# EricSteinberger/PokerRL

Measured on NVIDIA H100. Metric: CFR+ iterations/s, higher is better.
Workload: dtype f32

## Files before the change

### include/pokerrl_b200.h

```cpp
#ifndef POKERRL_B200_H
#define POKERRL_B200_H

#include <stdint.h>

#ifdef __cplusplus
extern "C" {
#endif

typedef void* prl_stream_t;

#define PRL_ABI_VERSION 10

enum {
    PRL_KIND_P0 = 0,
    PRL_KIND_P1 = 1,
    PRL_KIND_CHANCE = 2,
    PRL_KIND_FOLD = 3,
    PRL_KIND_SHOWDOWN = 4,
    PRL_KIND_SHOWDOWN_ALLIN = 5
};

enum { PRL_ALGO_VANILLA = 0, PRL_ALGO_CFR_PLUS = 1, PRL_ALGO_LINEAR = 2, PRL_ALGO_DCFR = 3, PRL_ALGO_PCFR_PLUS = 4 };

enum {
    PRL_STRAT_F32 = 0,
    PRL_STRAT_UNIFORM64 = 1,
    PRL_STRAT_AVG_F64 = 2,
    PRL_STRAT_AVG_SUM = 3,
    PRL_STRAT_AVG_F32 = 4
};

typedef struct {
    int32_t n_nodes, n_levels, n_slots;
    int32_t n_range;
    int32_t ld;
    int32_t n_hole;
    int32_t n_deck;
    int32_t n_suits;
    int32_t pair_bonus;
    int32_t max_actions;
    const int64_t* level_start;
    const int32_t* parent;
    const int32_t* first_child;
    const int32_t* n_children;
    const int32_t* slot;
    const int8_t* kind;
    const int8_t* acted_last;
    const float* pot;
    const int32_t* board;
    const int32_t* order;
    const int64_t* level_nonterm;
    const void* meta;
    const int64_t* level_ndec;
    const int8_t* hand_cards;
    int32_t n_boards;
    int32_t max_chance_children;
    const uint64_t* board_mask;
    const float* board_prob;
    const float* board_mult;
    const int16_t* board_gs;
    const int16_t* board_ge;
    const int16_t* board_pos;
    const int16_t* board_row_order;
    const uint8_t* board_row_pos;
    const uint8_t* board_complete;
    int32_t n_sym;
    const int16_t* sym_perm;
    float eq_const;
    const void* board_hand_rec;
    const void* node_rec2;
    const void* work_rec2;
    const int64_t* level_nfold;
    const int64_t* level_nallin;
    const int32_t* allin_nodes;
    const float* allin_pot;
    const void* const* allin_tiles;
    float* allin_partial;
} prl_tree_t;

typedef struct {
    float* reach;
    float* ev;
    float* ev_br;
    float* regret;
    float* strat;
    void* avg;
    void* workspace;
    uint64_t workspace_bytes;
    const float* dcfr;
} prl_buffers_t;

int prl_abi_version(void);
const char* prl_last_error(void);
unsigned long long prl_launch_count(void);

int prl_pack_node_meta(const prl_tree_t* tree, void* out_meta, prl_stream_t stream);

int prl_reach_pass(const prl_tree_t* tree, const prl_buffers_t* buf, int player_mask, const int* strat_mode,
                   prl_stream_t stream);

int prl_value_pass(const prl_tree_t* tree, const prl_buffers_t* buf, int player_mask, int with_br,
                   const int* strat_mode, prl_stream_t stream);

int prl_root_exploitability(const prl_tree_t* tree, const prl_buffers_t* buf, float* out_expl, prl_stream_t stream);

int prl_cfr_half_iteration(const prl_tree_t* tree, const prl_buffers_t* buf, int algo, int p, int iter, int delay,
                           int avg_f64, const int* strat_mode, prl_stream_t stream);

int prl_cfr_iterations(const prl_tree_t* tree, const prl_buffers_t* buf, int algo, int iter0, int n_iters, int delay,
                       int avg_f64, const int* strat_mode, prl_stream_t stream);

int prl_evaluate(const prl_tree_t* tree, const prl_buffers_t* buf, const int* strat_mode, int do_reach, float* out_expl,
                 prl_stream_t stream);

void prl_debug_set_timeline(void* device_u64_buffer);

int prl_cfr_sweep(const prl_tree_t* tree, const prl_buffers_t* buf, int algo, int p, int iter, int delay, int avg_f64,
                  const int* strat_mode, int which, prl_stream_t stream);

int prl_value_levels(const prl_tree_t* tree, const prl_buffers_t* buf, int player_mask, int with_br, int algo, int upd_p,
                     int iter, int delay, const int* strat_mode, int level_hi, int level_lo, int chance_phase,
                     prl_stream_t stream);
int prl_reach_update(const prl_tree_t* tree, const prl_buffers_t* buf, int algo, int p, int iter, int delay,
                     prl_stream_t stream);

int prl_reach_levels(const prl_tree_t* tree, const prl_buffers_t* buf, int player_mask, int algo, int upd_p, int iter,
                     int delay, const int* strat_mode, int level_lo, int level_hi, prl_stream_t stream);

int prl_gather_agent_policy(const float* probs, int n_actions, const int32_t* dec_of_slot, const int32_t* action_of_slot,
                            int n_slots, int n_range, int ld, float* out, prl_stream_t stream);

int prl_board_order_tables(const int32_t* ranks, int n_boards, int n_range, int n_deck, int16_t* gs, int16_t* ge,
                           int16_t* pos, int16_t* row_order, uint8_t* row_pos, prl_stream_t stream);

typedef struct {
    int32_t n_boards;
    int32_t n_range;
    int32_t ld;
    int32_t n_deck;
    int32_t n_local;
    int32_t frac_bits;
    int32_t grid;
    float eq_const;
    int8_t kind[16], parent[16], first_child[16], n_children[16], acted_last[16];
    float pot[16];
    int64_t row0[16];
    int32_t row_m[16];
    const void* tables;
    const float* board_prob;
    const float* board_mult;
    float* regret;
    float* avg;
    int64_t* w_private;
    int64_t* w_total;
    const float* dcfr;
    float* pred;
    float* rnr_reach;
    float rnr_p;
} prl_board_game_t;

int prl_board_layout(const prl_board_game_t* shape, int32_t* out);
int prl_board_grid(void);
int prl_board_shape_ok(const prl_board_game_t* g);
int prl_board_rows(const prl_board_game_t* shape, int32_t* row_of, int32_t* rows_per_board);

int prl_board_build_tables(const int32_t* ranks, const uint64_t* board_mask, const int8_t* hand_cards, int n_boards,
                           void* blob, prl_stream_t stream);

int prl_board_sweep(const prl_board_game_t* g, int p, int eval, int src_own, int src_opp, const float* trunk_reach_opp,
                    int iter, int delay, int algo, float defer_w, int p1_only, prl_stream_t stream);

int prl_board_update_cfrp(const prl_board_game_t* g, int p, const float* trunk_reach_opp, int iter, int delay, int due, int now,
                          prl_stream_t stream);
int prl_board_avg_flush(const prl_board_game_t* g, int p, int due, int delay, prl_stream_t stream);

int prl_board_collect(const prl_board_game_t* g, int n_arr, const int16_t* sym_perm, int n_sym, float* out, int ld,
                      prl_stream_t stream);

typedef struct {
    int32_t n_nodes, chance_node, n_buf_nodes, ld, n_range;
    int32_t mode[2];
    float eq_const;
    int8_t kind[8], first_child[8], n_children[8], acted_last[8];
    int32_t first_slot[8];
    float pot[8];
    const int8_t* hand_cards;
    float* reach;
    float* ev;
    float* ev_br;
    float* regret;
    float* strat;
    float* avg;
    const float* reach_model;
    float rnr_p;
} prl_trunk_t;

int prl_board_trunk(const prl_board_game_t* g, const prl_trunk_t* t, int eval, int p, int n_sym, const int16_t* sym_perm, int iter,
                    int delay, float* out_expl, const int64_t* const* peers, int n_peers, int64_t peer_offset, int64_t* w_scratch,
                    int algo, prl_stream_t stream);

int prl_board_permute(const prl_board_game_t* g, int rows_per_board, const int64_t* row_src, const int64_t* row_dst,
                      float* sorted_tab, float* natural_tab, int ld, int to_natural, prl_stream_t stream);

int prl_board_policy_query(const prl_board_game_t* shape, const float* rows, const int64_t* keys, const int16_t* pos_hand,
                           int n_cls, int iso, const int8_t* boards, int n_boards, const int32_t* out_index, uint64_t actions,
                           int n_actions, float* out, int32_t* miss, prl_stream_t stream);


int64_t prl_allin_tiles_bytes(int n_range);
int64_t prl_allin_partial_bytes(int n_range);
int prl_allin_equity_accumulate(const int32_t* ranks, const double* weight, int n_boards, int n_range, double* ec,
                                prl_stream_t stream);
int prl_allin_equity_finish(const double* ec, int n_range, const int8_t* hand_cards, const int16_t* sym_perm, int n_sym,
                            void* tiles, prl_stream_t stream);
int prl_allin_values(const void* tiles, int n_range, const float* const* x_rows, float* const* y_rows, float* const* y2_rows,
                     const float* scale, int n_cols, float* partial, prl_stream_t stream);

int prl_hand_rank_boards(const int8_t* boards, int n_boards, int32_t* out, prl_stream_t stream);

int prl_hand_rank_7(const int8_t* cards, int n, int32_t* out, prl_stream_t stream);

long long prl_lbr_workspace_doubles(int n_queries, int n_dealt);
int prl_lbr_checkdown_equity(const int8_t* lbr_hands, const int8_t* boards, int n_dealt, const float* ranges, int n_queries,
                             int first_board_ranks, double* workspace, float* out, prl_stream_t stream);

int32_t get_hand_rank_52_holdem(int8_t** hand_2d , int8_t** board_2d );
void get_hand_rank_all_hands_on_given_boards_52_holdem(int32_t** out , int8_t** boards_1d ,
                                                       int32_t n, int8_t** idx2holecards, int8_t** card1d_to_2d);
void get_hole_card_2_idx_lut(int16_t** lut );
void get_idx_2_hole_card_lut(int8_t** lut );
void get_idx_2_flop_lut(int8_t** lut );
void get_idx_2_turn_lut(int8_t** lut );
void get_idx_2_river_lut(int8_t** lut );
int8_t get_1d_card(const int8_t* card_2d);
void get_2d_card(int8_t card_1d, int8_t* out_card_2d);

#define PRL_ENV_MAX_ACTIONS 34

typedef struct {
    int32_t n_envs;
    int32_t kind;
    int32_t n_actions;
    int32_t n_rounds;
    int32_t n_round_slots;
    int32_t n_hole, n_ranks, n_suits, n_deck;
    int32_t n_flop, n_turn, n_river;
    int32_t small_blind, big_blind, ante, small_bet, big_bet, round_big_bet_starts;
    int32_t max_raises[4];
    int32_t first_action_no_call, limit_raise_is_pot, btn_first_postflop, suits_matter;
    int32_t pair_bonus;
    int32_t start_stack[2];
    int32_t obs_size;
    double fracs[32];
    double reward_scalar;
    double norm;
} prl_env_cfg_t;

int prl_env_state_fields(void);

int prl_env_reset(const prl_env_cfg_t* cfg, int32_t* state, int8_t* deck, float* obs, uint8_t* legal, uint64_t seed,
                  uint64_t episode0, int shuffle, prl_stream_t stream);

int prl_env_step(const prl_env_cfg_t* cfg, int32_t* state, int8_t* deck, const int32_t* actions, float* obs,
                 double* rewards, uint8_t* done, uint8_t* legal, uint64_t seed, uint64_t step_id, int auto_reset,
                 prl_stream_t stream);

#ifdef __cplusplus
}
#endif
#endif
```

### pokerrl_b200/_native.py

```python
import ctypes as C
import os

_HERE = os.path.dirname(os.path.abspath(__file__))
LIB_PATH = os.environ.get("PRL_LIB_PATH") or os.path.join(_HERE, "lib", "libpokerrl_b200.so")

KIND_P0, KIND_P1, KIND_CHANCE, KIND_FOLD, KIND_SHOWDOWN, KIND_SHOWDOWN_ALLIN = range(6)
ALGO_VANILLA, ALGO_CFR_PLUS, ALGO_LINEAR, ALGO_DCFR, ALGO_PCFR_PLUS = 0, 1, 2, 3, 4
ABI_VERSION = 10
STRAT_F32, STRAT_UNIFORM64, STRAT_AVG_F64, STRAT_AVG_SUM, STRAT_AVG_F32 = range(5)


class PrlTree(C.Structure):
    _fields_ = [
        ("n_nodes", C.c_int32), ("n_levels", C.c_int32), ("n_slots", C.c_int32), ("n_range", C.c_int32),
        ("ld", C.c_int32), ("n_hole", C.c_int32), ("n_deck", C.c_int32), ("n_suits", C.c_int32),
        ("pair_bonus", C.c_int32), ("max_actions", C.c_int32),
        ("level_start", C.c_void_p),
        ("parent", C.c_void_p), ("first_child", C.c_void_p), ("n_children", C.c_void_p), ("slot", C.c_void_p),
        ("kind", C.c_void_p), ("acted_last", C.c_void_p), ("pot", C.c_void_p), ("board", C.c_void_p),
        ("order", C.c_void_p), ("level_nonterm", C.c_void_p), ("meta", C.c_void_p),
        ("level_ndec", C.c_void_p), ("hand_cards", C.c_void_p), ("n_boards", C.c_int32),
        ("max_chance_children", C.c_int32), ("board_mask", C.c_void_p), ("board_prob", C.c_void_p),
        ("board_mult", C.c_void_p), ("board_gs", C.c_void_p), ("board_ge", C.c_void_p), ("board_pos", C.c_void_p),
        ("board_row_order", C.c_void_p), ("board_row_pos", C.c_void_p), ("board_complete", C.c_void_p),
        ("n_sym", C.c_int32), ("sym_perm", C.c_void_p), ("eq_const", C.c_float), ("board_hand_rec", C.c_void_p),
        ("node_rec2", C.c_void_p), ("work_rec2", C.c_void_p), ("level_nfold", C.c_void_p),
        ("level_nallin", C.c_void_p), ("allin_nodes", C.c_void_p), ("allin_pot", C.c_void_p), ("allin_tiles", C.c_void_p),
        ("allin_partial", C.c_void_p),
    ]


class PrlBuffers(C.Structure):
    _fields_ = [("reach", C.c_void_p), ("ev", C.c_void_p), ("ev_br", C.c_void_p), ("regret", C.c_void_p),
                ("strat", C.c_void_p), ("avg", C.c_void_p), ("workspace", C.c_void_p),
                ("workspace_bytes", C.c_uint64), ("dcfr", C.c_void_p)]


class PrlBoardGame(C.Structure):
    _fields_ = [("n_boards", C.c_int32), ("n_range", C.c_int32), ("ld", C.c_int32), ("n_deck", C.c_int32),
                ("n_local", C.c_int32), ("frac_bits", C.c_int32), ("grid", C.c_int32), ("eq_const", C.c_float),
                ("kind", C.c_int8 * 16), ("parent", C.c_int8 * 16), ("first_child", C.c_int8 * 16),
                ("n_children", C.c_int8 * 16), ("acted_last", C.c_int8 * 16), ("pot", C.c_float * 16),
                ("row0", C.c_int64 * 16), ("row_m", C.c_int32 * 16),
                ("tables", C.c_void_p), ("board_prob", C.c_void_p), ("board_mult", C.c_void_p), ("regret", C.c_void_p),
                ("avg", C.c_void_p), ("w_private", C.c_void_p), ("w_total", C.c_void_p), ("dcfr", C.c_void_p), ("pred", C.c_void_p),
                ("rnr_reach", C.c_void_p), ("rnr_p", C.c_float)]


class PrlTrunk(C.Structure):
    _fields_ = [("n_nodes", C.c_int32), ("chance_node", C.c_int32), ("n_buf_nodes", C.c_int32), ("ld", C.c_int32),
                ("n_range", C.c_int32), ("mode", C.c_int32 * 2), ("eq_const", C.c_float),
                ("kind", C.c_int8 * 8), ("first_child", C.c_int8 * 8), ("n_children", C.c_int8 * 8), ("acted_last", C.c_int8 * 8),
                ("first_slot", C.c_int32 * 8), ("pot", C.c_float * 8), ("hand_cards", C.c_void_p), ("reach", C.c_void_p),
                ("ev", C.c_void_p), ("ev_br", C.c_void_p), ("regret", C.c_void_p), ("strat", C.c_void_p), ("avg", C.c_void_p),
                ("reach_model", C.c_void_p), ("rnr_p", C.c_float)]


class PrlEnvCfg(C.Structure):
    _fields_ = [
        ("n_envs", C.c_int32), ("kind", C.c_int32), ("n_actions", C.c_int32), ("n_rounds", C.c_int32),
        ("n_round_slots", C.c_int32), ("n_hole", C.c_int32), ("n_ranks", C.c_int32), ("n_suits", C.c_int32),
        ("n_deck", C.c_int32), ("n_flop", C.c_int32), ("n_turn", C.c_int32), ("n_river", C.c_int32),
        ("small_blind", C.c_int32), ("big_blind", C.c_int32), ("ante", C.c_int32), ("small_bet", C.c_int32),
        ("big_bet", C.c_int32), ("round_big_bet_starts", C.c_int32), ("max_raises", C.c_int32 * 4),
        ("first_action_no_call", C.c_int32), ("limit_raise_is_pot", C.c_int32), ("btn_first_postflop", C.c_int32),
        ("suits_matter", C.c_int32), ("pair_bonus", C.c_int32), ("start_stack", C.c_int32 * 2), ("obs_size", C.c_int32),
        ("fracs", C.c_double * 32), ("reward_scalar", C.c_double), ("norm", C.c_double),
    ]


_lib = None


def lib():
    global _lib
    if _lib is not None:
        return _lib
    if not os.path.exists(LIB_PATH):
        raise RuntimeError(
            "pokerrl_b200: CUDA library %s is missing. Build it with `python -m pokerrl_b200.csrc.build` "
            "(or __graft_entry__.build()). There is no CPU fallback." % LIB_PATH)
    L = C.CDLL(LIB_PATH)
    L.prl_abi_version.restype = C.c_int
    if L.prl_abi_version() != ABI_VERSION:
        raise RuntimeError("pokerrl_b200: %s was built for ABI %d, the Python side expects %d - rebuild it with "
                           "`python -m pokerrl_b200.csrc.build`" % (LIB_PATH, L.prl_abi_version(), ABI_VERSION))
    L.prl_last_error.restype = C.c_char_p
    tp, bp, ip = C.POINTER(PrlTree), C.POINTER(PrlBuffers), C.POINTER(C.c_int)
    L.prl_reach_pass.argtypes = [tp, bp, C.c_int, ip, C.c_void_p]
    L.prl_value_pass.argtypes = [tp, bp, C.c_int, C.c_int, ip, C.c_void_p]
    L.prl_root_exploitability.argtypes = [tp, bp, C.c_void_p, C.c_void_p]
    L.prl_cfr_half_iteration.argtypes = [tp, bp, C.c_int, C.c_int, C.c_int, C.c_int, C.c_int, ip, C.c_void_p]
    L.prl_cfr_sweep.argtypes = [tp, bp, C.c_int, C.c_int, C.c_int, C.c_int, C.c_int, ip, C.c_int, C.c_void_p]
    L.prl_launch_count.restype = C.c_ulonglong
    L.prl_cfr_iterations.argtypes = [tp, bp, C.c_int, C.c_int, C.c_int, C.c_int, C.c_int, ip, C.c_void_p]
    L.prl_evaluate.argtypes = [tp, bp, ip, C.c_int, C.c_void_p, C.c_void_p]
    L.prl_pack_node_meta.argtypes = [tp, C.c_void_p, C.c_void_p]
    for f in ("prl_reach_pass", "prl_value_pass", "prl_root_exploitability", "prl_cfr_half_iteration", "prl_cfr_sweep", "prl_pack_node_meta", "prl_cfr_iterations",
              "prl_evaluate"):
        getattr(L, f).restype = C.c_int
    L.prl_value_levels.argtypes = [tp, bp, C.c_int, C.c_int, C.c_int, C.c_int, C.c_int, C.c_int, ip, C.c_int, C.c_int,
                                   C.c_int, C.c_void_p]
    L.prl_reach_update.argtypes = [tp, bp, C.c_int, C.c_int, C.c_int, C.c_int, C.c_void_p]
    L.prl_value_levels.restype = L.prl_reach_update.restype = C.c_int
    L.prl_reach_levels.argtypes = [tp, bp, C.c_int, C.c_int, C.c_int, C.c_int, C.c_int, ip, C.c_int, C.c_int, C.c_void_p]
    L.prl_reach_levels.restype = C.c_int
    L.prl_board_order_tables.argtypes = [C.c_void_p, C.c_int, C.c_int, C.c_int, C.c_void_p, C.c_void_p, C.c_void_p,
                                         C.c_void_p, C.c_void_p, C.c_void_p]
    L.prl_board_order_tables.restype = C.c_int
    L.prl_hand_rank_boards.argtypes = [C.c_void_p, C.c_int, C.c_void_p, C.c_void_p]
    L.prl_hand_rank_7.argtypes = [C.c_void_p, C.c_int, C.c_void_p, C.c_void_p]
    for f in ("prl_hand_rank_boards", "prl_hand_rank_7"):
        getattr(L, f).restype = C.c_int
    L.prl_gather_agent_policy.argtypes = [C.c_void_p, C.c_int, C.c_void_p, C.c_void_p, C.c_int, C.c_int, C.c_int, C.c_void_p,
                                          C.c_void_p]
    L.prl_gather_agent_policy.restype = C.c_int
    L.prl_lbr_workspace_doubles.argtypes = [C.c_int, C.c_int]
    L.prl_lbr_workspace_doubles.restype = C.c_longlong
    L.prl_lbr_checkdown_equity.argtypes = [C.c_void_p, C.c_void_p, C.c_int, C.c_void_p, C.c_int, C.c_int, C.c_void_p, C.c_void_p,
                                           C.c_void_p]
    L.prl_lbr_checkdown_equity.restype = C.c_int
    L.prl_allin_tiles_bytes.argtypes = L.prl_allin_partial_bytes.argtypes = [C.c_int]
    L.prl_allin_tiles_bytes.restype = L.prl_allin_partial_bytes.restype = C.c_int64
    L.prl_allin_equity_accumulate.argtypes = [C.c_void_p, C.c_void_p, C.c_int, C.c_int, C.c_void_p, C.c_void_p]
    L.prl_allin_equity_finish.argtypes = [C.c_void_p, C.c_int, C.c_void_p, C.c_void_p, C.c_int, C.c_void_p, C.c_void_p]
    L.prl_allin_values.argtypes = [C.c_void_p, C.c_int, C.c_void_p, C.c_void_p, C.c_void_p, C.c_void_p, C.c_int, C.c_void_p,
                                   C.c_void_p]
    for f in ("prl_allin_equity_accumulate", "prl_allin_equity_finish", "prl_allin_values"):
        getattr(L, f).restype = C.c_int
    gp = C.POINTER(PrlBoardGame)
    L.prl_board_layout.argtypes = [gp, C.POINTER(C.c_int32)]
    L.prl_board_grid.argtypes = []
    L.prl_board_rows.argtypes = [gp, C.POINTER(C.c_int32), C.POINTER(C.c_int32)]
    L.prl_board_rows.restype = C.c_int
    L.prl_board_shape_ok.argtypes = [gp]
    L.prl_board_build_tables.argtypes = [C.c_void_p, C.c_void_p, C.c_void_p, C.c_int, C.c_void_p, C.c_void_p]
    L.prl_board_sweep.argtypes = [gp, C.c_int, C.c_int, C.c_int, C.c_int, C.c_void_p, C.c_int, C.c_int, C.c_int, C.c_float, C.c_int,
                                  C.c_void_p]
    L.prl_board_update_cfrp.argtypes = [gp, C.c_int, C.c_void_p, C.c_int, C.c_int, C.c_int, C.c_int, C.c_void_p]
    L.prl_board_avg_flush.argtypes = [gp, C.c_int, C.c_int, C.c_int, C.c_void_p]
    L.prl_board_collect.argtypes = [gp, C.c_int, C.c_void_p, C.c_int, C.c_void_p, C.c_int, C.c_void_p]
    L.prl_board_permute.argtypes = [gp, C.c_int, C.c_void_p, C.c_void_p, C.c_void_p, C.c_void_p, C.c_int, C.c_int,
                                    C.c_void_p]
    L.prl_board_trunk.argtypes = [gp, C.POINTER(PrlTrunk), C.c_int, C.c_int, C.c_int, C.c_void_p, C.c_int, C.c_int, C.c_void_p,
                                  C.c_void_p, C.c_int, C.c_int64, C.c_void_p, C.c_int, C.c_void_p]
    L.prl_board_trunk.restype = C.c_int
    L.prl_board_policy_query.argtypes = [gp, C.c_void_p, C.c_void_p, C.c_void_p, C.c_int, C.c_int, C.c_void_p, C.c_int,
                                         C.c_void_p, C.c_uint64, C.c_int, C.c_void_p, C.c_void_p, C.c_void_p]
    for f in ("prl_board_layout", "prl_board_grid", "prl_board_shape_ok", "prl_board_build_tables", "prl_board_sweep",
              "prl_board_update_cfrp", "prl_board_avg_flush", "prl_board_collect", "prl_board_permute", "prl_board_policy_query"):
        getattr(L, f).restype = C.c_int
    ep = C.POINTER(PrlEnvCfg)
    L.prl_env_state_fields.restype = C.c_int
    L.prl_env_reset.argtypes = [ep, C.c_void_p, C.c_void_p, C.c_void_p, C.c_void_p, C.c_uint64, C.c_uint64, C.c_int,
                                C.c_void_p]
    L.prl_env_step.argtypes = [ep, C.c_void_p, C.c_void_p, C.c_void_p, C.c_void_p, C.c_void_p, C.c_void_p, C.c_void_p,
                               C.c_uint64, C.c_uint64, C.c_int, C.c_void_p]
    L.prl_env_reset.restype = L.prl_env_step.restype = C.c_int
    _lib = L
    return L


def call(name, *args):
    L = lib()
    rc = getattr(L, name)(*args)
    if rc != 0:
        raise RuntimeError("%s failed (%d): %s" % (name, rc, L.prl_last_error().decode()))


def modes(m0, m1):
    return (C.c_int * 2)(m0, m1)
```

### pokerrl_b200/board_engine.py

```python
import ctypes as C
import math
import os

import numpy as np
import torch

from pokerrl_b200 import _native as nat
from pokerrl_b200 import algorithm
from pokerrl_b200 import dcfr as _dcfr
from pokerrl_b200.game.flat_tree import FlatTree
from pokerrl_b200.game.holdem_boards import BoardSpec
from pokerrl_b200.solver import DeviceTree, TreeBuffers, TreeOps, _require_cuda

SRC_REGRET, SRC_AVG, SRC_AVG_SUM = 0, 1, 2


def board_layout(g=None):
    out = (C.c_int32 * 8)()
    nat.call("prl_board_layout", C.byref(g) if g is not None else None, out)
    return dict(n_live=out[0], ldb=out[1], blob=out[2], sh_off=out[3], rows_off=out[4], live_cards=out[5],
                row_pad=out[6], n_local=out[7])


def _stream(dev):
    return C.c_void_p(torch.cuda.current_stream(dev).cuda_stream)


def supports(game_cls, env_args, algo):
    if algo not in algorithm.ALL or game_cls.RULES.N_HOLE_CARDS != 2 or game_cls.RULES.N_CARDS_IN_DECK != 52:
        return False
    if game_cls.RULES.N_FLOP_CARDS != 5 or os.environ.get("PRL_ENGINE", "board") != "board":
        return False
    try:
        ft1 = FlatTree(game_cls, env_args, board_spec=_one_board_spec())
    except Exception:
        return False
    st = ft1.board_subtree()
    if st is None or sum(1 for n in ft1.abs_nodes if n.kind == nat.KIND_CHANCE) != 1:
        return False
    g = nat.PrlBoardGame()
    _fill_shape(g, st)
    return bool(nat.lib().prl_board_shape_ok(C.byref(g)))


def _one_board_spec():
    return BoardSpec(np.array([[0, 1, 2, 3, 4]], np.int8), np.ones(1), np.ones(1), None, "shape probe")


def _fill_shape(g, st):
    g.n_local = st["n_local"]
    for i in range(st["n_local"]):
        g.kind[i], g.parent[i], g.first_child[i] = st["kind"][i], st["parent"][i], st["first_child"][i]
        g.n_children[i], g.acted_last[i], g.pot[i] = st["n_children"][i], st["acted_last"][i], st["pot"][i]


def shape_rows(g):
    row_of, rpb = (C.c_int32 * 16)(), C.c_int32(0)
    nat.call("prl_board_rows", C.byref(g), row_of, C.byref(rpb))
    return list(row_of), int(rpb.value)


def board_mask(boards):
    mask = np.zeros(boards.shape[0], np.uint64)
    for k in range(boards.shape[1]):
        mask |= (np.uint64(1) << boards[:, k].astype(np.uint64))
    return mask


def build_board_blobs(rules, boards, t_blob, dev):
    from pokerrl_b200.hand_eval import hand_rank_all_hands_on_given_boards
    boards = np.ascontiguousarray(boards, np.int8)
    nb = boards.shape[0]
    lut = rules.get_lut_holder()
    t_hc = torch.from_numpy(np.ascontiguousarray(lut.LUT_IDX_2_HOLE_CARDS, np.int8)).to(dev)
    t_mask = torch.from_numpy(board_mask(boards).view(np.int64)).to(dev)
    CH = 16384
    for i in range(0, nb, CH):
        n = min(CH, nb - i)
        ranks = hand_rank_all_hands_on_given_boards(boards[i:i + n], device=dev)
        nat.call("prl_board_build_tables", C.c_void_p(ranks.data_ptr()), C.c_void_p(t_mask[i:i + n].data_ptr()),
                 C.c_void_p(t_hc.data_ptr()), n, C.c_void_p(t_blob[i:i + n].data_ptr()), _stream(dev))


def _decision_locals(st):
    return [i for i in range(st["n_local"]) if st["kind"][i] <= 1 and st["n_children"][i] > 0]


def board_game(st, rules, n_boards, ld, n_sym, grid=0):
    g = nat.PrlBoardGame()
    _fill_shape(g, st)
    g.n_boards, g.n_range, g.ld, g.n_deck = n_boards, rules.RANGE_SIZE, ld, rules.N_CARDS_IN_DECK
    n_hole = rules.N_HOLE_CARDS
    g.eq_const = math.comb(g.n_deck, n_hole) / math.comb(g.n_deck - n_hole, n_hole)
    bound = max(n_sym, 1) * g.eq_const * max(st["pot"]) * 0.5 * 4.0
    g.frac_bits = 62 - int(math.ceil(math.log2(bound)))
    n_local = st["n_local"]
    dec = _decision_locals(st)
    rows_per_board = sum(st["n_children"][i] for i in dec)
    row_of, rpb = shape_rows(g)
    assert rpb == rows_per_board
    local_rows = {}
    for i in range(n_local):
        g.row0[i], g.row_m[i] = -1, 0
    for d in dec:
        for a in range(st["n_children"][d]):
            c = st["first_child"][d] + a
            g.row0[c], g.row_m[c] = row_of[c], rpb
            local_rows[c] = (int(row_of[c]), rpb)
    g.grid = int(grid) if grid else int(nat.lib().prl_board_grid())
    return g, rows_per_board, local_rows


def row_map(local_rows, ft=None):
    st = None if ft is None else ft.board_subtree()
    src, dst = [], []
    for k, (i, (r0, m)) in enumerate(sorted(local_rows.items())):
        src += [r0, m]
        dst += [k, len(local_rows)] if ft is None else [int(ft.slot[st["node_base"][i] + st["node_k"][i]]), st["node_m"][i]]
    return src, dst


def _normalised(x, dim, matching):
    if matching:
        x = x.clamp(min=0)
    tot = x.sum(dim=dim, keepdim=True)
    ok = (tot > 0) if matching else (tot != 0)
    return torch.where(ok, x / torch.where(ok, tot, torch.ones_like(tot)), torch.full_like(x, 1.0 / x.shape[dim]))


def _sum_to_one(x, dim):
    d = x.double()
    tot = d.sum(dim=dim, keepdim=True)
    ok = tot > 0
    return torch.where(ok, d / torch.where(ok, tot, torch.ones_like(tot)), torch.full_like(d, 1.0 / d.shape[dim])).to(x.dtype)


def _decision_row_groups(st, local_rows):
    return [[local_rows[c][0] for c in range(st["first_child"][d], st["first_child"][d] + st["n_children"][d])]
            for d in _decision_locals(st)]


def _trunk_decisions(ft, chance_node):
    return [(int(ft.first_slot[n]), int(ft.n_children[n])) for n in range(chance_node + 1)
            if ft.kind[n] <= 1 and ft.first_child[n] >= 0]


class _BoardEngine:

    def _setup(self, game_cls, env_args, spec, n_boards, grid=0):
        dev = self.device
        self.rules = game_cls.RULES
        self.ev_normalizer = game_cls.EV_NORMALIZER
        self.L = board_layout()
        self.ft1 = FlatTree(game_cls, env_args, board_spec=_one_board_spec())
        st = self.ft1.board_subtree()
        if st is None:
            raise ValueError("the game does not have ONE chance layer with a <= 16-node post-deal subtree")
        self.st = st
        self.chance_level = st["chance_level"]
        self.chance_node = st["chance_node"]
        self.R = self.rules.RANGE_SIZE
        self.trunk = DeviceTree(self.ft1, dev)
        self.trunk.desc.n_sym = 0
        self.trunk.desc.sym_perm = None
        self.bufs = TreeBuffers(self.trunk)
        self.ld = self.trunk.ld
        sp = spec.sym_perm
        self.n_sym = 0 if sp is None else int(sp.shape[0])
        self.t_sym = None if sp is None else torch.from_numpy(np.ascontiguousarray(sp, np.int16)).to(dev)
        g, self.rows_per_board, self.local_rows = board_game(st, self.rules, n_boards, self.ld, self.n_sym, grid)
        self.w_private = torch.zeros((g.grid, 2, self.R), dtype=torch.int64, device=dev)
        self._expl = torch.zeros(2, dtype=torch.float32, device=dev)
        g.w_private = self.w_private.data_ptr()
        self.g = g
        nb = self.n_boards_total = int(spec.boards.shape[0])
        self.n_nodes = int(self.ft1.level_start[self.chance_level + 1]) + nb * st["n_local"]
        self.n_nonterm = (int((self.ft1.kind[:self.chance_node + 1] <= nat.KIND_CHANCE).sum())
                          + nb * len(_decision_locals(st)))

    def _setup_boards(self, capacity):
        dev, n = self.device, max(capacity, 1)
        self.t_blob = torch.empty((n, self.L["blob"]), dtype=torch.uint8, device=dev)
        self.t_prob = torch.zeros(n, dtype=torch.float32, device=dev)
        self.t_mult = torch.zeros(n, dtype=torch.float32, device=dev)
        g = self.g
        g.tables, g.board_prob, g.board_mult = self.t_blob.data_ptr(), self.t_prob.data_ptr(), self.t_mult.data_ptr()

    def _load_boards(self, boards, prob, mult):
        n = boards.shape[0]
        build_board_blobs(self.rules, boards, self.t_blob, self.device)
        self.t_prob[:n].copy_(torch.from_numpy(np.ascontiguousarray(prob, np.float32)))
        self.t_mult[:n].copy_(torch.from_numpy(np.ascontiguousarray(mult, np.float32)))
        self.g.n_boards = n

    def _trunk_desc(self, bufs, modes):
        ft, t = self.ft1, nat.PrlTrunk()
        n = self.chance_node + 1
        assert n <= 8 and int(ft.level_start[self.chance_level + 1]) == n, "the trunk must be the first nodes of the flat tree"
        t.n_nodes, t.chance_node, t.n_buf_nodes, t.ld, t.n_range = n, self.chance_node, self.trunk.n_nodes, self.ld, self.R
        t.mode[0], t.mode[1] = modes
        t.eq_const = self.g.eq_const
        for i in range(n):
            t.kind[i], t.first_child[i], t.n_children[i] = int(ft.kind[i]), int(ft.first_child[i]), int(ft.n_children[i])
            t.acted_last[i], t.pot[i] = int(ft.acted_last[i]), float(ft.pot[i])
            t.first_slot[i] = int(ft.first_slot[i]) if ft.first_slot[i] >= 0 else 0
        t.hand_cards = self.trunk.t_hand_cards.data_ptr()
        t.reach, t.ev, t.ev_br = bufs.reach.data_ptr(), bufs.ev.data_ptr(), bufs.ev_br.data_ptr()
        t.regret, t.strat, t.avg = bufs.regret.data_ptr(), bufs.strat.data_ptr(), bufs.avg.data_ptr()
        return t

    def _trunk_reach_row(self, bufs, seat):
        return C.c_void_p(bufs.reach.data_ptr() + 4 * (seat * self.trunk.n_nodes + self.chance_node) * self.ld)

    def _reach_trunk(self, bufs, mask, algo, upd_p, modes, t, delay):
        nat.call("prl_reach_levels", C.byref(self.trunk.desc), C.byref(bufs.desc), mask, algo, upd_p, t, delay,
                 nat.modes(*modes), 0, self.chance_level, _stream(self.device))

    @property
    def n_trunk_slots(self):
        return self.ft1.n_slots - self.rows_per_board

    def _board_sweep(self, bufs, p, evaluate, src_own, src_opp, t, delay, algo, defer_w=0.0, p1_only=0):
        nat.call("prl_board_sweep", C.byref(self.g), p, int(evaluate), src_own, src_opp, self._trunk_reach_row(bufs, 1 - p),
                 t, delay, algo, defer_w, p1_only, _stream(self.device))

    def _board_trunk(self, bufs, modes, evaluate, p, t, delay, algo, peers=None, n_peers=0, peer_off=0, w_scratch=None):
        nat.call("prl_board_trunk", C.byref(self.g), C.byref(self._trunk_desc(bufs, modes)), int(evaluate), p, self.n_sym,
                 C.c_void_p(self.t_sym.data_ptr()) if self.n_sym else None, t, delay, C.c_void_p(self._expl.data_ptr()), peers,
                 n_peers, peer_off, w_scratch, algo, _stream(self.device))

    def _board_permute(self, tab, nat_tab, to_natural, ft=None, lo=0, hi=None):
        g = self.g
        if hi is not None:
            g = nat.PrlBoardGame.from_buffer_copy(self.g)
            g.n_boards, g.tables = hi - lo, self.t_blob[lo].data_ptr()
        src, dst = (torch.tensor(x, dtype=torch.int64, device=self.device) for x in row_map(self.local_rows, ft))
        nat.call("prl_board_permute", C.byref(g), len(self.local_rows), C.c_void_p(src.data_ptr()), C.c_void_p(dst.data_ptr()),
                 C.c_void_p(tab[lo * self.rows_per_board].data_ptr()), C.c_void_p(nat_tab.data_ptr()), self.ld, to_natural,
                 _stream(self.device))


class BoardCFRSolver(_BoardEngine):
    def __init__(self, game_cls, env_args, board_spec=None, algo="CFRPlus", delay=0, device=None, rank=0, world=1,
                 group=None, grid=0, reduce_fn=None, dcfr=_dcfr.DEFAULT, pcfr_gamma=algorithm.PCFR_GAMMA):
        self.device = _require_cuda(device)
        self.alg = algorithm.Algorithm(algo, delay, dcfr, self.device, pcfr_gamma)
        self.algo_name, self.algo, self.delay, self.dcfr = self.alg.name, self.alg.code, self.alg.delay, self.alg.dcfr
        self._factors = self.alg.factors
        self.rank, self.world, self.group = int(rank), int(world), group
        self._reduce_fn = reduce_fn
        self.game_cls, self.env_args = game_cls, env_args
        spec = board_spec if board_spec is not None else BoardSpec.full_game(game_cls.RULES)
        self.spec_full = spec
        with torch.cuda.device(self.device):
            self._build(spec, grid)
        self.n_allreduce = 0
        self.reset()

    def _build(self, spec, grid):
        dev = self.device
        sel = np.arange(self.rank, spec.boards.shape[0], self.world)
        self.board_ids = sel
        self.boards = np.ascontiguousarray(spec.boards[sel], np.int8)
        nb = self.n_boards = int(sel.size)
        self._setup(self.game_cls, self.env_args, spec, nb, grid)
        self.ops = TreeOps(self.trunk, self.bufs)
        self._eval_bufs = None
        self._setup_boards(nb)
        self._load_boards(self.boards, spec.board_prob[sel], spec.board_mult[sel])
        torch.cuda.synchronize(dev)
        g = self.g
        self.n_rows = nb * self.rows_per_board
        self.regret = torch.zeros((max(self.n_rows, 1), self.L["ldb"]), dtype=torch.float32, device=dev)
        self.avg = torch.zeros_like(self.regret)
        g.regret, g.avg = self.regret.data_ptr(), self.avg.data_ptr()
        self.pred = torch.zeros_like(self.regret) if self.algo == nat.ALGO_PCFR_PLUS else None
        g.pred = self.pred.data_ptr() if self.pred is not None else None
        self._symm = None
        self.collective = "none" if self.world == 1 else "nccl all_reduce(int64)"
        if (self.world > 1 and self._reduce_fn is None and os.environ.get("PRL_COLLECTIVE", "p2p") == "p2p"
                and os.environ.get("PRL_TRUNK", "fused") != "levels"):
            try:
                import torch.distributed as dist
                import torch.distributed._symmetric_memory as symm_mem
                self.w_gens = symm_mem.empty((2, 4, self.R), dtype=torch.int64, device=dev)
                self.w_gens.zero_()
                self._symm = symm_mem.rendezvous(self.w_gens, group=self.group if self.group is not None else dist.group.WORLD)
                self._peer_ptrs = torch.tensor([int(x) for x in self._symm.buffer_ptrs], dtype=torch.int64, device=dev)
                self.collective = "one-shot NVLink sum inside trunk_kernel (symmetric memory, %d peers)" % self.world
            except Exception as e:
                self._symm = None
                self.collective = "nccl all_reduce(int64) (symmetric memory unavailable: %s)" % type(e).__name__
        if self._symm is None:
            self.w_gens = torch.zeros((2, 4, self.R), dtype=torch.int64, device=dev)
        self._gen = 0
        self.w_total = self.w_gens[0]
        self.w_scratch = torch.zeros((4, self.R), dtype=torch.int64, device=dev)
        g.w_total = self.w_total.data_ptr()
        self.fused_trunk = os.environ.get("PRL_TRUNK", "fused") != "levels"
        self._w_off = 4 * self.ld

    def _clear_pending(self):
        self._pending = [0.0, 0.0]
        self._avg_due = [-1, -1]

    def _trunk(self, bufs, modes, evaluate, p):
        peers, n_peers, off = None, 0, 0
        if self._symm is not None:
            peers, n_peers, off = C.c_void_p(self._peer_ptrs.data_ptr()), self.world, self._gen * 4 * self.R
        self._board_trunk(bufs, modes, evaluate, p, self.iter_counter, self.delay, self.algo, peers, n_peers, off,
                          C.c_void_p(self.w_scratch.data_ptr()))

    def _board_update_cfrp(self, p, due, now):
        nat.call("prl_board_update_cfrp", C.byref(self.g), p, self._trunk_reach_row(self.bufs, 1 - p), self.iter_counter,
                 self.delay, due, now, _stream(self.device))

    def _next_generation(self):
        self._gen ^= 1
        self.w_total = self.w_gens[self._gen]
        self.g.w_total = self.w_total.data_ptr()

    def _reduce(self, view):
        if self._symm is not None:
            self._symm.barrier(channel=0)
            self.n_allreduce += 1
            return
        if self._reduce_fn is not None:
            self._reduce_fn(view)
        elif self.world > 1:
            import torch.distributed as dist
            dist.all_reduce(view, op=dist.ReduceOp.SUM, group=self.group)
        self.n_allreduce += 1

    def _levels(self, bufs, mask, with_br, algo, upd_p, modes, hi, lo, phase):
        nat.call("prl_value_levels", C.byref(self.trunk.desc), C.byref(bufs.desc), mask, int(with_br), algo, upd_p,
                 self.iter_counter, self.delay, nat.modes(*modes), hi, lo, phase, _stream(self.device))

    def _sweep_begin(self, bufs, p, evaluate, src_own, src_opp):
        if not evaluate and self.algo == nat.ALGO_CFR_PLUS:
            t, due = self.iter_counter, self._avg_due[p]
            now = 1 if due >= 0 or t < self.delay else 0
            self._avg_due[p] = -1 if now else t
            self._board_update_cfrp(p, due, now)
            return
        defer_w = 0.0
        if not evaluate and self.algo != nat.ALGO_CFR_PLUS:
            defer_w, self._pending[1 - p] = self._pending[1 - p], 0.0
        self._board_sweep(bufs, p, evaluate, src_own, src_opp, self.iter_counter, self.delay, self.algo, defer_w)

    def flush_average(self):
        with torch.cuda.device(self.device):
            for q in (0, 1):
                if self._avg_due[q] >= 0:
                    nat.call("prl_board_avg_flush", C.byref(self.g), q, self._avg_due[q], self.delay, _stream(self.device))
                    self._avg_due[q] = -1
                if self._pending[q] != 0.0:
                    self._board_sweep(self.bufs, 1 - q, False, 0, 0, self.iter_counter, self.delay, self.algo,
                                      defer_w=self._pending[q], p1_only=1)
                    self._pending[q] = 0.0

    def _sweep_end(self, bufs, p, evaluate):
        n_arr = 2 if evaluate else 1
        view = self.w_total[2 * p:2 * p + 2] if evaluate else self.w_total[:1]
        self._reduce(view)
        out = bufs.workspace.data_ptr() + 4 * (self._w_off + 2 * p * self.ld)
        g2 = self.g
        if evaluate and p == 1:
            g2 = nat.PrlBoardGame.from_buffer_copy(self.g)
            g2.w_total = self.w_total.data_ptr() + 8 * 2 * self.R
        nat.call("prl_board_collect", C.byref(g2), n_arr, C.c_void_p(self.t_sym.data_ptr()) if self.n_sym else None,
                 self.n_sym, C.c_void_p(out), self.ld, _stream(self.device))

    def _sweep(self, bufs, p, evaluate, src_own, src_opp):
        self._sweep_begin(bufs, p, evaluate, src_own, src_opp)
        self._sweep_end(bufs, p, evaluate)

    def _update_begin(self, p):
        cl = self.chance_level
        self.g.dcfr = self.alg.factor_table(self.iter_counter + 1)
        if not self.fused_trunk:
            self._levels(self.bufs, 1 << p, False, self.algo, p, self.modes, cl, cl, 1)
        self._sweep_begin(self.bufs, p, False, SRC_REGRET, SRC_REGRET)

    def _update_end(self, p):
        cl = self.chance_level
        if self.algo != nat.ALGO_CFR_PLUS:
            if not self.fused_trunk:
                raise RuntimeError("Vanilla / Linear CFR, DCFR and PCFR+ on the board engine need the fused trunk (unset "
                                   "PRL_TRUNK=levels)")
            self._pending[p] = self.alg.sum_weight(self.iter_counter)
        if self.fused_trunk:
            self._reduce(self.w_total[:1])
            self._trunk(self.bufs, self.modes, False, p)
            self.modes[p] = nat.STRAT_F32
            self._next_generation()
            return
        self._sweep_end(self.bufs, p, False)
        self._levels(self.bufs, 1 << p, False, self.algo, p, self.modes, cl, cl, 2)
        if cl > 0:
            self._levels(self.bufs, 1 << p, False, self.algo, p, self.modes, cl - 1, 0, 0)
        self.modes[p] = nat.STRAT_F32
        self._reach_trunk(self.bufs, 1 << p, self.algo, p, self.modes, self.iter_counter, self.delay)

    def reset(self):
        with torch.cuda.device(self.device):
            self.iter_counter = 0
            for t in (self.regret, self.avg, self.bufs.regret, self.bufs.strat, self.bufs.avg):
                t.zero_()
            if self.pred is not None:
                self.pred.zero_()
            self._clear_pending()
            self.modes = [nat.STRAT_UNIFORM64, nat.STRAT_UNIFORM64]
            self._reach_trunk(self.bufs, 3, -1, -1, self.modes, self.iter_counter, self.delay)

    def iteration(self, n=1):
        with torch.cuda.device(self.device):
            for _ in range(n):
                for p in (0, 1):
                    self._update_begin(p)
                    self._update_end(p)
                self.iter_counter += 1

    def _evaluate(self, bufs, modes, src):
        cl = self.chance_level
        if self.fused_trunk:
            for p in (0, 1):
                self._sweep_begin(bufs, p, True, src, src)
            self._reduce(self.w_total)
            self._trunk(bufs, modes, True, -1)
            self._next_generation()
            e = self._expl.cpu().numpy()
        else:
            self._levels(bufs, 3, True, -1, -1, modes, cl, cl, 1)
            for p in (0, 1):
                self._sweep(bufs, p, True, src, src)
            self._levels(bufs, 3, True, -1, -1, modes, cl, cl, 2)
            if cl > 0:
                self._levels(bufs, 3, True, -1, -1, modes, cl - 1, 0, 0)
            e = (TreeOps(self.trunk, bufs) if bufs is not self.bufs else self.ops).root_exploitability()
        return algorithm.seat_averaged(e, self.ev_normalizer)

    def exploitability_current(self):
        with torch.cuda.device(self.device):
            return self._evaluate(self.bufs, self.modes, SRC_REGRET)

    def exploitability_average(self):
        if self.iter_counter == 0:
            raise RuntimeError("no average strategy before the first iteration")
        m, src = {algorithm.SUMS: (nat.STRAT_AVG_SUM, SRC_AVG_SUM), algorithm.CURRENT: (nat.STRAT_F32, SRC_REGRET),
                  algorithm.AVERAGE: (nat.STRAT_AVG_F32, SRC_AVG)}[self.alg.average(self.iter_counter)]
        with torch.cuda.device(self.device):
            if self._eval_bufs is None:
                self._eval_bufs = TreeBuffers(self.trunk, share=self.bufs)
            self.flush_average()
            self._reach_trunk(self._eval_bufs, 3, -1, -1, [m, m], self.iter_counter, self.delay)
            return self._evaluate(self._eval_bufs, [m, m], src)

    def natural_tables(self, ft):
        assert ft.board_spec.boards.shape[0] == self.n_boards
        self.flush_average()
        nts, out = self.n_trunk_slots, []
        pairs = [(self.regret, self.bufs.regret), (self.avg, self.bufs.avg)]
        if self.pred is not None:
            pairs.append((self.pred, self.bufs.strat))
        with torch.cuda.device(self.device):
            for tab, trunk_tab in pairs:
                nat_tab = torch.zeros((ft.n_slots, self.ld), dtype=torch.float32, device=self.device)
                self._board_permute(tab, nat_tab, 1, ft)
                nat_tab[:nts] = trunk_tab[:nts]
                out.append(nat_tab)
        return out

    def load_natural_tables(self, ft, regret, avg, pred=None):
        if (pred is None) != (self.pred is None):
            raise ValueError("load_natural_tables: predictions are given exactly for PCFR+")
        self._clear_pending()
        nts, dev = self.n_trunk_slots, self.device
        triples = [(self.regret, self.bufs.regret, regret), (self.avg, self.bufs.avg, avg)]
        if pred is not None:
            triples.append((self.pred, None, pred))
        with torch.cuda.device(dev):
            for tab, trunk_tab, given in triples:
                nat_tab = torch.zeros((ft.n_slots, self.ld), dtype=torch.float32, device=dev)
                nat_tab[:, :given.shape[1]] = torch.as_tensor(given, dtype=torch.float32).to(dev)
                self._board_permute(tab, nat_tab, 0, ft)
                if trunk_tab is not None:
                    trunk_tab[:nts] = nat_tab[:nts]
                else:
                    self._set_trunk_strategy(nat_tab)

    def set_trunk_strategy_from_regrets(self):
        if self.pred is not None:
            raise RuntimeError("PCFR+: the trunk strategy is regret matching of the predictions given to load_natural_tables")
        self._set_trunk_strategy(self.bufs.regret)

    def _set_trunk_strategy(self, rows):
        ft = self.ft1
        for n in range(self.chance_node + 1):
            if ft.kind[n] <= 1 and ft.first_child[n] >= 0:
                fs, A = int(ft.first_slot[n]), int(ft.n_children[n])
                self.bufs.strat[fs:fs + A] = _normalised(rows[fs:fs + A], 0, True)
        self.modes = [nat.STRAT_F32, nat.STRAT_F32]
        with torch.cuda.device(self.device):
            self._reach_trunk(self.bufs, 3, -1, -1, self.modes, self.iter_counter, self.delay)

    def _identity(self):
        return {"engine": "board", **self.alg.identity(), "rank": self.rank, "world": self.world, "n_boards": self.n_boards,
                "n_boards_total": self.n_boards_total}

    def state_dict(self):
        self.flush_average()
        return {**self._identity(), "iter_counter": self.iter_counter, "modes": list(self.modes),
                "regret": self.regret.cpu(), "avg": self.avg.cpu(),
                "trunk_regret": self.bufs.regret.cpu(), "trunk_strat": self.bufs.strat.cpu(), "trunk_avg": self.bufs.avg.cpu(),
                **({"pred": self.pred.cpu()} if self.alg.code == nat.ALGO_PCFR_PLUS else {})}

    def load_state_dict(self, state):
        algorithm.check_identity(state, self._identity())
        if tuple(state["regret"].shape) != tuple(self.regret.shape):
            raise ValueError("checkpoint table shape %s != %s" % (tuple(state["regret"].shape), tuple(self.regret.shape)))
        self.iter_counter, self.modes = int(state["iter_counter"]), list(state["modes"])
        self._clear_pending()
        self.regret.copy_(state["regret"])
        self.avg.copy_(state["avg"])
        if self.alg.code == nat.ALGO_PCFR_PLUS:
            self.pred.copy_(state["pred"])
        self.bufs.regret.copy_(state["trunk_regret"])
        self.bufs.strat.copy_(state["trunk_strat"])
        self.bufs.avg.copy_(state["trunk_avg"])
        with torch.cuda.device(self.device):
            self._reach_trunk(self.bufs, 3, -1, -1, self.modes, self.iter_counter, self.delay)


def rnr_probability(p):
    p = float(p)
    if not (math.isfinite(p) and 0.0 <= p <= 1.0):
        raise ValueError("the model's probability p must be a finite number in [0, 1], got %r" % p)
    return float(np.float32(p))


def rnr_identity(seat, p, model_digest):
    return {"rnr_seat": int(seat), "rnr_p": float(p), "rnr_model": model_digest}


def device_digest(tensors):
    acc, mask = 0, (1 << 61) - 1
    for k, t in enumerate(tensors):
        flat = t.reshape(-1).view(torch.int32)
        for a in range(0, flat.numel(), 1 << 24):
            v = flat[a:a + (1 << 24)].to(torch.int64)
            w = torch.arange(a + 1, a + 1 + v.numel(), dtype=torch.int64, device=t.device) * 2654435761 + k
            acc = (acc * 1000003 + int((v * w).sum())) & mask
    return acc


class BoardRNRSolver(BoardCFRSolver):

    def __init__(self, game_cls, env_args, seat, p, board_spec=None, delay=0, device=None, grid=0, share_boards=None):
        if seat not in (0, 1):
            raise ValueError("the exploiter's seat is 0 or 1")
        self.seat, self.p = int(seat), rnr_probability(p)
        if self.p > 0.0 and os.environ.get("PRL_TRUNK", "fused") == "levels":
            raise ValueError("the restricted Nash response needs the fused trunk (unset PRL_TRUNK=levels)")
        self._q = float(np.float32(1.0) - np.float32(self.p))
        self._rnr_trunk = False
        self._share = share_boards
        super().__init__(game_cls, env_args, board_spec, algo="CFRPlus", delay=delay, device=device, grid=grid)
        dev = self.device
        self.n_sd = sum(1 for k in self.st["kind"][:self.st["n_local"]] if k == nat.KIND_SHOWDOWN)
        self.model_reach = torch.zeros((max(self.n_boards * self.n_sd, 1), self.L["ldb"]), dtype=torch.float32, device=dev)
        self.trunk_model = torch.zeros_like(self.bufs.reach)
        self.model_digest = None
        self._opp_row = torch.zeros(self.ld, dtype=torch.float32, device=dev)
        self._expl = torch.zeros(6, dtype=torch.float32, device=dev)

    def _setup_boards(self, capacity):
        if self._share is None:
            return super()._setup_boards(capacity)
        sh = self._share
        if sh.n_boards != capacity or not np.array_equal(sh.boards, self.boards) or sh.device != self.device:
            raise ValueError("share_boards: another board spec or device")
        self.t_blob, self.t_prob, self.t_mult = sh.t_blob, sh.t_prob, sh.t_mult
        self.g.tables, self.g.board_prob, self.g.board_mult = sh.g.tables, sh.g.board_prob, sh.g.board_mult

    def _load_boards(self, boards, prob, mult):
        if self._share is None:
            return super()._load_boards(boards, prob, mult)
        self.g.n_boards = boards.shape[0]

    def set_model(self, trunk_model):
        self.trunk_model.copy_(trunk_model)
        with torch.cuda.device(self.device):
            self.model_digest = device_digest([self.model_reach, self.trunk_model])

    def _rnr_game(self, p):
        g = nat.PrlBoardGame.from_buffer_copy(self.g)
        g.rnr_reach, g.rnr_p = self.model_reach.data_ptr(), p
        return g

    def _skipped(self, p):
        return p != self.seat and self.p == 1.0

    def _board_update_cfrp(self, p, due, now):
        if p != self.seat or self.p == 0.0:
            return super()._board_update_cfrp(p, due, now)
        free = self.bufs.reach.view(2, -1, self.ld)[1 - p, self.chance_node]
        torch.mul(free, self._q, out=self._opp_row)
        nat.call("prl_board_update_cfrp", C.byref(self._rnr_game(self.p)), p, C.c_void_p(self._opp_row.data_ptr()),
                 self.iter_counter, self.delay, due, now, _stream(self.device))

    def _trunk(self, bufs, modes, evaluate, p):
        self._rnr_trunk = not evaluate and p == self.seat and self.p > 0.0
        try:
            super()._trunk(bufs, modes, evaluate, p)
        finally:
            self._rnr_trunk = False

    def _trunk_desc(self, bufs, modes):
        t = super()._trunk_desc(bufs, modes)
        if self._rnr_trunk:
            t.reach_model, t.rnr_p = self.trunk_model.data_ptr(), self.p
        return t

    def _update_begin(self, p):
        if not self._skipped(p):
            super()._update_begin(p)

    def _update_end(self, p):
        if not self._skipped(p):
            super()._update_end(p)

    def rnr_values(self):
        if self.model_digest is None:
            raise RuntimeError("the model's tables are not set")
        if self.iter_counter == 0:
            raise RuntimeError("no average strategy before the first iteration")
        m, src = {algorithm.CURRENT: (nat.STRAT_F32, SRC_REGRET),
                  algorithm.AVERAGE: (nat.STRAT_AVG_F32, SRC_AVG)}[self.alg.average(self.iter_counter)]
        s, o = self.seat, 1 - self.seat
        with torch.cuda.device(self.device):
            if self._eval_bufs is None:
                self._eval_bufs = TreeBuffers(self.trunk, share=self.bufs)
            self.flush_average()
            bufs = self._eval_bufs
            self._reach_trunk(bufs, 3, -1, -1, [m, m], self.iter_counter, self.delay)
            bufs.reach[o].copy_(self.trunk_model[o])
            self._opp_row.zero_()
            nat.call("prl_board_sweep", C.byref(self._rnr_game(1.0)), s, 1, src, src, C.c_void_p(self._opp_row.data_ptr()),
                     self.iter_counter, self.delay, nat.ALGO_CFR_PLUS, 0.0, 0, _stream(self.device))
            self._board_sweep(bufs, o, True, src, src, self.iter_counter, self.delay, nat.ALGO_CFR_PLUS)
            self._reduce(self.w_total)
            self._rnr_trunk = True
            try:
                self._board_trunk(bufs, [m, m], True, -1, self.iter_counter, self.delay, nat.ALGO_CFR_PLUS)
            finally:
                self._rnr_trunk = False
            self._next_generation()
            e = self._expl.cpu().numpy().astype(np.float64)
        return float(e[2 + s]), float(e[4 + o])

    def _identity(self):
        return {**super()._identity(), **rnr_identity(self.seat, self.p, self.model_digest)}


def board_keys(boards):
    b = np.sort(np.asarray(boards, np.int64), axis=1)
    key = np.zeros(b.shape[0], np.int64)
    for i in range(b.shape[1]):
        key = key * 64 + b[:, i]
    return key


def abstract_fingerprint(ft):
    import hashlib
    a = np.array([(n.kind, n.action, n.pot, len(n.children), n.parent, n.acted_last) for n in ft.abs_nodes], np.int64)
    return hashlib.sha1(a.tobytes()).hexdigest()


class BoardPolicyEvaluator(_BoardEngine):

    MAX_CHUNK = 65536

    def __init__(self, env_bldr, stack_size=None, board_spec=None, chunk=None, device=None):
        self.device = dev = _require_cuda(device)
        self.env_bldr, self.stack_size = env_bldr, stack_size
        game_cls = env_bldr.env_cls
        self.env_args = env_bldr.args_for_stack(stack_size)
        self.spec = board_spec if board_spec is not None else BoardSpec.full_game(game_cls.RULES)
        n_actions = env_bldr.N_ACTIONS
        with torch.cuda.device(dev):
            self._setup(game_cls, self.env_args, self.spec, 0)
            L, rpb, g = self.L, self.rows_per_board, self.g
            n_dec = len(_decision_locals(self.st))
            self.bytes_per_board = (L["blob"] + rpb * L["ldb"] * 4 + rpb * self.ld * 4 + n_dec * self.R * n_actions * 4
                                    + self.R * 4)
            if chunk is None:
                free, _ = torch.cuda.mem_get_info(dev)
                chunk = min(self.MAX_CHUNK, free // 2 // self.bytes_per_board)
            self.chunk = max(1, min(int(chunk), self.n_boards_total))
            n = self.chunk
            self._setup_boards(n)
            self.rows = torch.zeros((n * rpb, L["ldb"]), dtype=torch.float32, device=dev)
            self.nat_tab = torch.zeros((self.n_trunk_slots + n * rpb, self.ld), dtype=torch.float32, device=dev)
            self.w_total = torch.zeros((4, self.R), dtype=torch.int64, device=dev)
            self.w_acc = torch.zeros_like(self.w_total)
            g.regret = g.avg = self.rows.data_ptr()
            g.w_total = self.w_total.data_ptr()
        self.times = {}

    def _chunk_tree(self, lo, hi):
        from pokerrl_b200.game.PublicTree import PublicTree
        s = self.spec
        spec = BoardSpec(s.boards[lo:hi], s.board_prob[lo:hi], s.board_mult[lo:hi], s.sym_perm,
                         "boards %d .. %d of: %s" % (lo, hi, s.note))
        pt = PublicTree(self.env_bldr, self.stack_size, stop_at_street=None, put_out_new_round_after_limit=True,
                        device=self.device, board_spec=spec)
        pt.build_structure()
        return pt

    def _chunks(self, agent, tick, normalise=False):
        import time
        R, s, nts = self.R, self.spec, self.n_trunk_slots
        for lo in range(0, self.n_boards_total, self.chunk):
            hi = min(lo + self.chunk, self.n_boards_total)
            t0 = time.perf_counter()
            pt = self._chunk_tree(lo, hi)
            ft = pt.flat
            tab = self.nat_tab[:ft.n_slots]
            got = pt.agent_strategy_table(agent, out=tab)
            if not isinstance(got, torch.Tensor):
                tab[:, :R].copy_(torch.from_numpy(np.ascontiguousarray(got, np.float32)))
            t0 = tick("agent query", t0)
            self._load_boards(s.boards[lo:hi], s.board_prob[lo:hi], s.board_mult[lo:hi])
            self._board_permute(self.rows, tab, 0, ft)
            if normalise:
                rows = self.rows[:(hi - lo) * self.rows_per_board].view(hi - lo, self.rows_per_board, -1)[:, :, :self.L["n_live"]]
                for idx in _decision_row_groups(self.st, self.local_rows):
                    rows[:, idx] = _sum_to_one(rows[:, idx], 1)
            if lo == 0:
                self.bufs.avg[:nts].copy_(tab[:nts])
                if normalise:
                    for fs, A in _trunk_decisions(self.ft1, self.chance_node):
                        self.bufs.avg[fs:fs + A, :R] = _sum_to_one(self.bufs.avg[fs:fs + A, :R], 0)
                self._reach_trunk(self.bufs, 3, -1, -1, [nat.STRAT_AVG_F32, nat.STRAT_AVG_F32], 0, 0)
            t0 = tick("table build", t0)
            yield lo, hi, t0
            del pt

    def model_reach(self, agent, tables):
        n_sd = sum(1 for k in self.st["kind"][:self.st["n_local"]] if k == nat.KIND_SHOWDOWN)
        with torch.cuda.device(self.device):
            for lo, hi, _ in self._chunks(agent, lambda key, t0: t0, normalise=True):
                for seat, F in tables.items():
                    g = nat.PrlBoardGame.from_buffer_copy(self.g)
                    g.rnr_reach, g.rnr_p = F[lo * n_sd].data_ptr(), 1.0
                    nat.call("prl_board_sweep", C.byref(g), seat, 0, SRC_AVG, SRC_AVG,
                             self._trunk_reach_row(self.bufs, 1 - seat), 0, 0, nat.ALGO_CFR_PLUS, 0.0, 1, _stream(self.device))
            return self.bufs.reach.clone()

    def evaluate(self, agent, profile=False):
        import time
        dev = self.device
        times = {"agent query": 0.0, "table build": 0.0, "sweeps": 0.0}
        modes = [nat.STRAT_AVG_F32, nat.STRAT_AVG_F32]

        def tick(key, t0):
            if profile:
                torch.cuda.synchronize(dev)
                t1 = time.perf_counter()
                times[key] += t1 - t0
                return t1
            return t0

        with torch.cuda.device(dev):
            self.w_acc.zero_()
            for lo, hi, t0 in self._chunks(agent, tick):
                for p in (0, 1):
                    self._board_sweep(self.bufs, p, True, SRC_AVG, SRC_AVG, 0, 0, nat.ALGO_CFR_PLUS)
                    self.w_acc[2 * p:2 * p + 2] += self.w_total[2 * p:2 * p + 2]
                tick("sweeps", t0)
            t0 = time.perf_counter()
            self.w_total.copy_(self.w_acc)
            self._board_trunk(self.bufs, modes, True, -1, 0, 0, nat.ALGO_CFR_PLUS)
            e = self._expl.cpu().numpy().astype(np.float64)
            tick("sweeps", t0)
        self.times = times
        return e


class BoardPolicyTables:

    def __init__(self, rows, keys, pos_hand, trunk, iso, actions, fingerprint, spec_id):
        self.rows, self.keys, self.pos_hand, self.trunk = rows, keys, pos_hand, trunk
        self.iso, self.actions, self.fingerprint, self.spec_id = bool(iso), int(actions), fingerprint, spec_id
        self.n_cls = int(keys.shape[0])
        self.rows_per_board = int(rows.shape[0]) // self.n_cls

    @classmethod
    def from_solver(cls, s):
        import hashlib
        if s.world != 1:
            raise ValueError("a sharded solver holds only its rank's boards")
        s.flush_average()
        avg = s.alg.average(s.iter_counter)
        nb, rpb, st = s.n_boards, s.rows_per_board, s.st
        groups = _decision_row_groups(st, s.local_rows)
        with torch.cuda.device(s.device):
            if avg == algorithm.AVERAGE:
                rows = s.avg.clone()
            else:
                matching = avg == algorithm.CURRENT
                rows = torch.empty_like(s.avg)
                src = (s.regret if matching else s.avg).view(nb, rpb, -1)
                dst = rows.view(nb, rpb, -1)
                for lo in range(0, nb, 8192):
                    hi = min(lo + 8192, nb)
                    for idx in groups:
                        dst[lo:hi, idx] = _normalised(src[lo:hi, idx], 1, matching)
            nts, ft = s.n_trunk_slots, s.ft1
            if avg != algorithm.SUMS:
                trunk = (s.bufs.strat if avg == algorithm.CURRENT else s.bufs.avg)[:nts].clone()
            else:
                a = s.bufs.avg[:nts]
                trunk = torch.zeros_like(a)
                for n in range(s.chance_node + 1):
                    if ft.kind[n] <= 1 and ft.first_child[n] >= 0:
                        fs, A = int(ft.first_slot[n]), int(ft.n_children[n])
                        trunk[fs:fs + A] = _normalised(a[fs:fs + A], 0, False)
            L = s.L
            pos_hand = s.t_blob[:nb, L["sh_off"]:L["sh_off"] + 2 * L["n_live"]].contiguous().view(torch.int16)
            keys = board_keys(s.boards)
            if np.any(np.diff(keys) <= 0):
                perm = np.argsort(keys, kind="stable")
                t_perm = torch.from_numpy(perm).to(s.device)
                rows = rows.view(nb, rpb, -1)[t_perm].reshape(nb * rpb, -1)
                pos_hand = pos_hand[t_perm]
                keys = keys[perm]
            t_keys = torch.from_numpy(keys).to(s.device)
        spec_id = (int(nb), s.n_sym > 0, hashlib.sha1(keys.tobytes()).hexdigest())
        return cls(rows, t_keys, pos_hand, trunk, s.n_sym > 0, _packed_actions(s.ft1, st), abstract_fingerprint(s.ft1),
                   spec_id)

    def _check(self, ft):
        if abstract_fingerprint(ft) != self.fingerprint:
            raise ValueError("this agent's tables were computed on a different betting tree (game / stack / bet set)")

    def _query(self, st, boards, out_index, out, n_actions):
        g = nat.PrlBoardGame()
        _fill_shape(g, st)
        if shape_rows(g)[1] != self.rows_per_board:
            raise ValueError("this agent's tables hold %d rows per board, the queried tree's post-deal shape has %d"
                             % (self.rows_per_board, shape_rows(g)[1]))
        dev = out.device
        miss = torch.zeros(1, dtype=torch.int32, device=dev)
        t_b = torch.from_numpy(np.ascontiguousarray(boards, np.int8)).to(dev)
        t_i = torch.from_numpy(np.ascontiguousarray(out_index, np.int32)).to(dev)
        with torch.cuda.device(dev):
            nat.call("prl_board_policy_query", C.byref(g), C.c_void_p(self.rows.data_ptr()), C.c_void_p(self.keys.data_ptr()),
                     C.c_void_p(self.pos_hand.data_ptr()), self.n_cls, int(self.iso), C.c_void_p(t_b.data_ptr()), int(t_b.shape[0]),
                     C.c_void_p(t_i.data_ptr()), self.actions, n_actions, C.c_void_p(out.data_ptr()), C.c_void_p(miss.data_ptr()),
                     _stream(dev))
        if int(miss.item()):
            raise ValueError("a queried board is not in this agent's board spec (%s)"
                             % ("suit classes" if self.iso else "boards without isomorphism"))

    def answer_tree(self, ft, n_actions):
        self._check(ft)
        dev = self.rows.device
        dec = np.nonzero((ft.kind <= nat.KIND_P1) & (ft.first_child >= 0))[0]
        dec_idx = np.full(ft.n_nodes, -1, np.int64)
        dec_idx[dec] = np.arange(dec.size)
        out = torch.empty((dec.size, ft.R, n_actions), dtype=torch.float32, device=dev)
        for n in dec[ft.cdepth[dec] == 0]:
            self._trunk_node(ft, n, out[dec_idx[n]])
        st = ft.board_subtree()
        nb = int(st["n_boards_local"])
        J = np.arange(nb, dtype=np.int64)
        locs = _decision_locals(st)
        idx = np.full((nb, len(locs)), -1, np.int64)
        for d, i in enumerate(locs):
            idx[:, d] = dec_idx[st["node_base"][i] + J * st["node_m"][i] + st["node_k"][i]]
        self._query(st, ft.board_spec.boards, idx, out, n_actions)
        return out

    def answer_node(self, ft, n, n_actions):
        self._check(ft)
        out = torch.empty((1, ft.R, n_actions), dtype=torch.float32, device=self.rows.device)
        if ft.cdepth[n] == 0:
            self._trunk_node(ft, n, out[0])
            return out[0].cpu().numpy()
        st = ft.board_subtree()
        j = int(ft.board[n]) - int(st["first_board"])
        locs = _decision_locals(st)
        idx = np.full((1, len(locs)), -1, np.int64)
        for d, i in enumerate(locs):
            if st["node_base"][i] + j * st["node_m"][i] + st["node_k"][i] == n:
                idx[0, d] = 0
        assert (idx == 0).sum() == 1, "not a post-deal decision node"
        self._query(st, ft.board_spec.boards[j:j + 1], idx, out, n_actions)
        return out[0].cpu().numpy()

    def _trunk_node(self, ft, n, out):
        fs, fc, A = int(ft.first_slot[n]), int(ft.first_child[n]), int(ft.n_children[n])
        out.zero_()
        out[:, torch.from_numpy(ft.action[fc:fc + A].astype(np.int64)).to(out.device)] = self.trunk[fs:fs + A, :ft.R].T

    def state_dict(self):
        return {"rows": self.rows.cpu(), "keys": self.keys.cpu(), "pos_hand": self.pos_hand.cpu(), "trunk": self.trunk.cpu(),
                "iso": self.iso, "actions": self.actions, "fingerprint": self.fingerprint, "spec_id": self.spec_id}

    @classmethod
    def from_state(cls, state, device=None):
        dev = _require_cuda(device)
        return cls(*(state[k].to(dev) for k in ("rows", "keys", "pos_hand", "trunk")), state["iso"], state["actions"],
                   state["fingerprint"], state["spec_id"])


def _packed_actions(ft, st):
    act = 0
    for i in range(1, st["n_local"]):
        a = int(ft.action[st["node_base"][i] + st["node_k"][i]])
        assert 0 <= a < 16
        act |= a << (4 * i)
    return act
```

### pokerrl_b200/csrc/cfr_board.cu

```cuda
#include <cuda_runtime.h>
#include <stdint.h>
#include <type_traits>

#include "pokerrl_b200.h"
#include "prl_common.cuh"

namespace {

constexpr int kDeck = 52;
constexpr int kBoardCards = 5;
constexpr int kLiveCards = kDeck - kBoardCards;
constexpr int kLive = kLiveCards * (kLiveCards - 1) / 2;
constexpr int kLdb = 1088;
constexpr int kRowLen = kLiveCards - 1;
constexpr int kRowPad = 48;
constexpr int kRowSeg = 12;
constexpr int kErStride = kLiveCards;
constexpr int kZeroSlot = kLive + 1;
constexpr int kRange = 1326;

constexpr int kRecBytes = kLdb * 8;
constexpr int kShBytes = kLdb * 2;
constexpr int kRowIdxBytes = kLiveCards * kRowPad * 2;
constexpr int kBlobA = kRecBytes + kShBytes;
constexpr int kBlobBytes = kBlobA + kRowIdxBytes;
static_assert(kBlobA % 16 == 0 && kRowIdxBytes % 16 == 0, "bulk copies move multiples of 16 bytes");

#ifndef PRL_BV_STAMPS
#define PRL_BV_STAMPS 0
#endif

constexpr int kThreads = 384;
constexpr int kWarps = kThreads / 32;

struct Nodes15 {
    int v[15];
};
constexpr unsigned long long pack_nodes(Nodes15 t) {
    unsigned long long r = 0;
    for (int i = 0; i < 15; ++i) r |= (unsigned long long)(t.v[i] + 1) << (4 * i);
    return r;
}
constexpr int unpack_node(unsigned long long t, int i) { return (int)((t >> (4 * i)) & 0xF) - 1; }

template <class SH>
struct ShapeOps {
    static constexpr int kind(int i) { return unpack_node(SH::kKind, i); }
    static constexpr int parent(int i) { return unpack_node(SH::kParent, i); }
    static constexpr int first_child(int i) { return unpack_node(SH::kFirstChild, i); }
    static constexpr int n_children(int i) { return unpack_node(SH::kNChildren, i); }
    static constexpr int vec_index(int i) {
        int n = 0;
        for (int k = 0; k < i; ++k) n += (kind(k) == kind(i));
        return n;
    }
    static constexpr int count(int k) {
        int n = 0;
        for (int i = 0; i < SH::N; ++i) n += (kind(i) == k);
        return n;
    }
    static constexpr int rows_of_seat(int p) {
        int n = 0;
        for (int i = 1; i < SH::N; ++i) n += (kind(parent(i)) == p);
        return n;
    }
    static constexpr int row_of(int c) {
        const int p = kind(parent(c));
        int n = (p == 0) ? 0 : rows_of_seat(0);
        for (int k = 1; k < c; ++k) n += (kind(parent(k)) == p);
        return n;
    }
    static constexpr int n_dec() {
        int n = 0;
        for (int i = 0; i < SH::N; ++i) n += (kind(i) <= 1 && n_children(i) > 0);
        return n;
    }
    static constexpr int dec_node(int d) {
        int n = 0;
        for (int i = 0; i < SH::N; ++i)
            if (kind(i) <= 1 && n_children(i) > 0 && n++ == d) return i;
        return -1;
    }
};

struct ShapeFHP : ShapeOps<ShapeFHP> {
    static constexpr int N = 15;
    static constexpr unsigned long long kKind = pack_nodes({{1, 0, 0, 4, 1, 3, 4, 1, 3, 4, 0, 3, 4, 3, 4}});
    static constexpr unsigned long long kParent = pack_nodes({{-1, 0, 0, 1, 1, 2, 2, 2, 4, 4, 4, 7, 7, 10, 10}});
    static constexpr unsigned long long kFirstChild = pack_nodes({{1, 3, 5, -1, 8, -1, -1, 11, -1, -1, 13, -1, -1, -1, -1}});
    static constexpr unsigned long long kNChildren = pack_nodes({{2, 2, 3, 0, 3, 0, 0, 2, 0, 0, 2, 0, 0, 0, 0}});
    static constexpr int n_sd = 5, n_fold = 4;
    static constexpr int rows = 14;
    static constexpr int fold_coef(int P, int f, int v) {
        constexpr int c[2][4][5] = {{{0, 1, 0, 0, 0}, {1, 0, -1, 0, -1}, {0, 1, 0, -1, 0}, {0, 0, 0, 0, 1}},
                                    {{1, -1, 1, -1, 0}, {0, 0, 1, 0, 0}, {0, 0, 0, 1, 0}, {0, 0, 1, 0, -1}}};
        return c[P][f][v];
    }
};

struct ShapeFHPShort : ShapeOps<ShapeFHPShort> {
    static constexpr int N = 9;
    static constexpr unsigned long long kKind = pack_nodes({{1, 0, 0, 4, 1, 3, 4, 3, 4}});
    static constexpr unsigned long long kParent = pack_nodes({{-1, 0, 0, 1, 1, 2, 2, 4, 4}});
    static constexpr unsigned long long kFirstChild = pack_nodes({{1, 3, 5, -1, 7, -1, -1, -1, -1}});
    static constexpr unsigned long long kNChildren = pack_nodes({{2, 2, 2, 0, 2, 0, 0, 0, 0}});
    static constexpr int n_sd = 3, n_fold = 2;
    static constexpr int rows = 8;
    static constexpr int fold_coef(int P, int f, int v) {
        constexpr int c[2][2][3] = {{{0, 1, 0}, {1, 0, -1}}, {{1, -1, 1}, {0, 0, 1}}};
        return c[P][f][v];
    }
};

template <class SH>
constexpr bool shape_consistent() {
    return SH::count(4) == SH::n_sd && SH::count(3) == SH::n_fold && SH::rows_of_seat(0) + SH::rows_of_seat(1) == SH::rows &&
           SH::N <= 15 && SH::n_fold % 2 == 0;
}
static_assert(shape_consistent<ShapeFHP>() && shape_consistent<ShapeFHPShort>(), "shape");

template <int I, int N, class F>
__device__ __forceinline__ void static_for(F&& f) {
    if constexpr (I < N) {
        f(std::integral_constant<int, I>{});
        static_for<I + 1, N>(f);
    }
}
template <int I, int N, class F>
__device__ __forceinline__ void static_for_down(F&& f) {
    if constexpr (I < N) {
        f(std::integral_constant<int, N - 1>{});
        static_for_down<I, N - 1>(f);
    }
}

constexpr int kErVec = kLiveCards * kErStride;
template <class SH>
struct SweepSmem {
    static constexpr int kNVec = SH::n_sd + SH::n_fold;
    static constexpr int kSOff = 0;
    static constexpr int kErOff = kSOff + kNVec * kLdb * 4;
    static constexpr int kErBytes = ((SH::n_sd * kErVec * 4) + 15) & ~15;
    static constexpr int kBlobOff = kErOff + kErBytes;
    static constexpr int kRowIdxOff = kBlobOff + 2 * kBlobA;
    static constexpr int kCsOff = kRowIdxOff + kRowIdxBytes;
    static constexpr int kCsdOff = kCsOff + SH::n_fold * kRowPad * 4;
    static constexpr int kMiscOff = kCsdOff + SH::n_fold * kRowPad * 8;
    static constexpr int kMiscBytes = (SH::n_sd * 16 + SH::n_sd * 16) * 8 + 8 * 4;
    static constexpr int kRowTotOff = kMiscOff + kMiscBytes;
    static constexpr int kRowTotBytes = SH::n_sd * kRowPad * 8;
    static constexpr int kBarOff = kRowTotOff + kRowTotBytes;
    static constexpr int kSmemBytes = kBarOff + 32;
    static_assert(kBlobOff % 16 == 0 && kRowIdxOff % 16 == 0 && kCsdOff % 8 == 0 && kMiscOff % 8 == 0 && kRowTotOff % 8 == 0 &&
                      kBarOff % 8 == 0, "alignment");
    static_assert(2 * (kSmemBytes + 1024) <= 233472, "two CTAs per SM (228 KB of shared memory per H100 SM)");
    static_assert(SH::n_fold <= 8, "tf[8]");
};

struct SweepArgs {
    prl_board_game_t g;
    const float* trunk_reach_opp;
    int iter, delay;
    float m_old, m_new;
    int pair;
    float m_old_due, m_new_due;
    int src_own, src_opp;
    float rw;
    const float* disc;
    float defer_w;
    double fx_scale;
    float sc[16];
};

__device__ __forceinline__ uint32_t smem_u32(const void* p) { return (uint32_t)__cvta_generic_to_shared(p); }
__device__ __forceinline__ void mbar_init(uint64_t* bar, int count) {
    asm volatile("mbarrier.init.shared::cta.b64 [%0], %1;" ::"r"(smem_u32(bar)), "r"(count) : "memory");
}
__device__ __forceinline__ void mbar_expect_tx(uint64_t* bar, uint32_t bytes) {
    asm volatile("mbarrier.arrive.expect_tx.shared::cta.b64 _, [%0], %1;" ::"r"(smem_u32(bar)), "r"(bytes) : "memory");
}
__device__ __forceinline__ void bulk_g2s(void* dst, const void* src, uint32_t bytes, uint64_t* bar) {
    asm volatile("cp.async.bulk.shared::cluster.global.mbarrier::complete_tx::bytes [%0], [%1], %2, [%3];" ::"r"(smem_u32(dst)),
                 "l"(src), "r"(bytes), "r"(smem_u32(bar))
                 : "memory");
}
__device__ __forceinline__ void bulk_prefetch_l2(const void* src, uint32_t bytes) {
    asm volatile("cp.async.bulk.prefetch.L2.global [%0], %1;" ::"l"(src), "r"(bytes) : "memory");
}
__device__ __forceinline__ void mbar_wait(uint64_t* bar, uint32_t parity) {
    uint32_t ok;
    do {
        asm volatile(
            "{\n\t.reg .pred p;\n\tmbarrier.try_wait.parity.shared::cta.b64 p, [%1], %2;\n\tselp.u32 %0, 1, 0, p;\n\t}"
            : "=r"(ok)
            : "r"(smem_u32(bar)), "r"(parity)
            : "memory");
    } while (!ok);
}
__device__ __forceinline__ void fence_async_shared() { asm volatile("fence.proxy.async.shared::cta;" ::: "memory"); }

#if PRL_BV_STAMPS
constexpr int kStampCtas = 512, kStampUnits = 16, kStampEvery = 32, kStampSlots = 8;
__device__ long long g_stamps[kStampCtas * kStampUnits * kStampSlots];
#endif
__device__ __forceinline__ void stamp(int it, int slot) {
#if PRL_BV_STAMPS
    if (threadIdx.x == 0 && blockIdx.x < kStampCtas && it % kStampEvery == 0 && it / kStampEvery < kStampUnits) {
        long long* r = g_stamps + ((size_t)blockIdx.x * kStampUnits + it / kStampEvery) * kStampSlots;
        r[slot] = clock64();
        if (slot == 0) {
            unsigned smid;
            asm volatile("mov.u32 %0, %%smid;" : "=r"(smid));
            r[6] = smid;
            r[7] = it;
        }
    }
#endif
}

template <int A>
__device__ __forceinline__ void node_strategy(const float (&g)[A], int src, float (&s)[A]) {
    if (src == 1) {
#pragma unroll
        for (int a = 0; a < A; ++a) s[a] = g[a];
        return;
    }
    float sum = 0.0f;
#pragma unroll
    for (int a = 0; a < A; ++a) {
        s[a] = fmaxf(g[a], 0.0f);
        sum += s[a];
    }
    const bool pos = sum > 0.0f;
    const float sm = fmaxf(sum, 1e-37f);
    float inv;
    asm("rcp.approx.ftz.f32 %0, %1;" : "=f"(inv) : "f"(sm));
    inv = fmaf(inv, fmaf(-sm, inv, 1.0f), inv);
    inv = pos ? inv : 0.0f;
    const float uni = pos ? 0.0f : 1.0f / (float)A;
#pragma unroll
    for (int a = 0; a < A; ++a) s[a] = fmaf(s[a], inv, uni);
}

__device__ __forceinline__ float avg_step(float m_old, float avg, float m_new, float s) {
    return __fmaf_rn(m_old, avg, __fmul_rn(m_new, s));
}

__device__ __forceinline__ float ld_stream(const float* p) { return __ldcs(p); }
__device__ __forceinline__ void st_stream(float* p, float v) { __stcs(p, v); }

constexpr int kRnrMix = 1, kRnrOut = 2;
template <class SH, int P, bool EVAL, bool DEFER = false, bool P1ONLY = false, bool AVG = true, bool PRED = false, int RNR = 0>
__global__ void __launch_bounds__(kThreads, 2) board_sweep_kernel(const SweepArgs a) {
    static_assert(!(EVAL && DEFER) && (!P1ONLY || DEFER || RNR == kRnrOut) && (AVG || (!EVAL && !DEFER)), "variants");
    static_assert(!PRED || (DEFER && !P1ONLY), "PRED is an update form of the DEFER family");
    static_assert(RNR == 0 || (!DEFER && !PRED && (RNR == kRnrOut) == P1ONLY && (RNR == kRnrMix || !EVAL)), "RNR forms");
    using M = SweepSmem<SH>;
    constexpr int NSD = SH::n_sd, NF = SH::n_fold;
    extern __shared__ __align__(128) unsigned char smem[];
    float* S = reinterpret_cast<float*>(smem + M::kSOff);
    float* Er = reinterpret_cast<float*>(smem + M::kErOff);
    float* cs = reinterpret_cast<float*>(smem + M::kCsOff);
    double* csd = reinterpret_cast<double*>(smem + M::kCsdOff);
    double* wsum = reinterpret_cast<double*>(smem + M::kMiscOff);
    double* wexc = wsum + NSD * 16;
    float* tf = reinterpret_cast<float*>(wexc + NSD * 16);
    uint64_t* bars = reinterpret_cast<uint64_t*>(smem + M::kBarOff);
    const int16_t* rowidx = reinterpret_cast<const int16_t*>(smem + M::kRowIdxOff);
    double* rowtot = reinterpret_cast<double*>(smem + M::kRowTotOff);
    constexpr bool kLin = !EVAL;

    const int tid = threadIdx.x, lane = tid & 31, warp = tid >> 5;
    const prl_board_game_t& G = a.g;
    const int nb = G.n_boards;
    constexpr int OPP = 1 - P;
    constexpr int ROWS = SH::rows;
    constexpr int OWN0 = (P == 0) ? 0 : SH::rows_of_seat(0);
    constexpr int OPP0 = (P == 0) ? SH::rows_of_seat(0) : 0;
    constexpr int NOWN = SH::rows_of_seat(P), NOPP = SH::rows_of_seat(OPP);
    constexpr size_t kBoardFloats = (size_t)ROWS * kLdb;
    const unsigned char* blob_g = reinterpret_cast<const unsigned char*>(G.tables);
    const float* tab_opp = PRED ? G.pred : (RNR == kRnrOut || (EVAL && a.src_opp >= 1)) ? G.avg : G.regret;
    const float* tab_own = (EVAL && a.src_own >= 1) ? G.avg : G.regret;
    const int asis_opp = (RNR == kRnrOut || (EVAL && a.src_opp == 1)) ? 1 : 0, asis_own = (EVAL && a.src_own == 1) ? 1 : 0;
    constexpr size_t kRnrFloats = (size_t)SH::n_sd * kLdb;
    const bool do_avg = !EVAL && !DEFER && AVG && a.iter >= a.delay;
    const bool pair = do_avg && a.pair;
    const bool defer_now = DEFER && a.defer_w != 0.0f;
    float* disc = reinterpret_cast<float*>(smem + M::kBarOff + 3 * sizeof(uint64_t));
    const bool read_avg = do_avg && (pair ? a.m_old_due : a.m_old) != 0.0f;

    long long* wp = reinterpret_cast<long long*>(G.w_private) + (size_t)blockIdx.x * 2 * kRange;
    for (int h = tid; h < 2 * kRange; h += kThreads) wp[h] = 0;
    for (int v = 0; v < M::kNVec; ++v)
        for (int i = kLive + tid; i < kLdb; i += kThreads) S[v * kLdb + i] = 0.0f;
    if (tid == 0) {
        mbar_init(&bars[0], 1);
        mbar_init(&bars[1], 1);
        mbar_init(&bars[2], 1);
        fence_async_shared();
        if (DEFER && a.disc) {
            disc[0] = a.disc[0];
            disc[1] = a.disc[1];
        }
    }
    __syncthreads();
    int j = blockIdx.x;
    auto prefetch_rows = [&](int jj) {
        bulk_prefetch_l2(tab_opp + (size_t)jj * kBoardFloats + (size_t)OPP0 * kLdb, NOPP * kLdb * 4);
        bulk_prefetch_l2(tab_own + (size_t)jj * kBoardFloats + (size_t)OWN0 * kLdb, NOWN * kLdb * 4);
        if (read_avg) bulk_prefetch_l2(G.avg + (size_t)jj * kBoardFloats + (size_t)OWN0 * kLdb, NOWN * kLdb * 4);
        if (defer_now) bulk_prefetch_l2(G.avg + (size_t)jj * kBoardFloats + (size_t)OPP0 * kLdb, NOPP * kLdb * 4);
        if constexpr (RNR == kRnrMix) bulk_prefetch_l2(G.rnr_reach + (size_t)jj * kRnrFloats, kRnrFloats * 4);
    };
    constexpr bool kPfPhase = !EVAL;
    auto prefetch_opp = [&](int jj) {
        bulk_prefetch_l2(tab_opp + (size_t)jj * kBoardFloats + (size_t)OPP0 * kLdb, NOPP * kLdb * 4);
        if (defer_now) bulk_prefetch_l2(G.avg + (size_t)jj * kBoardFloats + (size_t)OPP0 * kLdb, NOPP * kLdb * 4);
        if constexpr (RNR == kRnrMix) bulk_prefetch_l2(G.rnr_reach + (size_t)jj * kRnrFloats, kRnrFloats * 4);
    };
    auto prefetch_own = [&](int jj) {
        bulk_prefetch_l2(tab_own + (size_t)jj * kBoardFloats + (size_t)OWN0 * kLdb, NOWN * kLdb * 4);
        if (read_avg) bulk_prefetch_l2(G.avg + (size_t)jj * kBoardFloats + (size_t)OWN0 * kLdb, NOWN * kLdb * 4);
        if constexpr (PRED) bulk_prefetch_l2(G.pred + (size_t)jj * kBoardFloats + (size_t)OWN0 * kLdb, NOWN * kLdb * 4);
    };
    if (tid == 0 && j < nb) {
        mbar_expect_tx(&bars[0], kBlobA);
        bulk_g2s(smem + M::kBlobOff, blob_g + (size_t)j * kBlobBytes, kBlobA, &bars[0]);
        if (!P1ONLY) {
            mbar_expect_tx(&bars[2], kRowIdxBytes);
            bulk_g2s(smem + M::kRowIdxOff, blob_g + (size_t)j * kBlobBytes + kBlobA, kRowIdxBytes, &bars[2]);
        }
        if constexpr (kPfPhase) prefetch_opp(j);
        else prefetch_rows(j);
    }

    float p1_g[NOPP], p1_x0;
    auto p1_load_k = [&](int jj, const int16_t* sh_jj, int k, float (&g)[NOPP], float& x0) {
        const int i = min(tid + k * kThreads, kLive - 1);
        const float* rows = tab_opp + (size_t)jj * kBoardFloats + (size_t)OPP0 * kLdb + i;
#pragma unroll
        for (int r = 0; r < NOPP; ++r) g[r] = ld_stream(rows + (size_t)r * kLdb);
        x0 = __ldg(a.trunk_reach_opp + sh_jj[i]);
    };
    auto p1_load = [&](int jj, const int16_t* sh_jj) { p1_load_k(jj, sh_jj, 0, p1_g, p1_x0); };

    for (int it = 0; j < nb; j += gridDim.x, ++it) {
        const int buf = it & 1;
        const unsigned char* blob = smem + M::kBlobOff + buf * kBlobA;
        const uint64_t* rec = reinterpret_cast<const uint64_t*>(blob);
        const int16_t* sh = reinterpret_cast<const int16_t*>(blob + kRecBytes);
        const int jn = j + gridDim.x;
        stamp(it, 0);
        if (tid == 0 && jn < nb) {
            mbar_expect_tx(&bars[buf ^ 1], kBlobA);
            bulk_g2s(smem + M::kBlobOff + (buf ^ 1) * kBlobA, blob_g + (size_t)jn * kBlobBytes, kBlobA, &bars[buf ^ 1]);
            if constexpr (!kPfPhase) prefetch_rows(jn);
        }
        const float prob = __ldg(G.board_prob + j);
        if (it == 0) {
            mbar_wait(&bars[buf], 0);
            p1_load(j, sh);
        }

        auto p1_hand = [&](int k, const float (&gk)[NOPP], float x0k) {
            const int i = tid + k * kThreads;
            if (i < kLive) {
                float x[SH::N];
                x[0] = x0k * prob;
                float fm[RNR == kRnrMix ? NSD : 1];
                if constexpr (RNR == kRnrMix) {
#pragma unroll
                    for (int v = 0; v < NSD; ++v) fm[v] = ld_stream(G.rnr_reach + (size_t)j * kRnrFloats + (size_t)v * kLdb + i);
                }
                static_for<0, SH::N>([&](auto I) {
                    constexpr int n = decltype(I)::value;
                    constexpr int A = SH::n_children(n);
                    if constexpr (SH::kind(n) <= 1) {
                        constexpr int fc = SH::first_child(n);
                        if constexpr (SH::kind(n) == OPP) {
                            constexpr int r0 = SH::row_of(fc);
                            float gg[A], s[A];
#pragma unroll
                            for (int c = 0; c < A; ++c) gg[c] = gk[r0 - OPP0 + c];
                            node_strategy<A>(gg, asis_opp, s);
#pragma unroll
                            for (int c = 0; c < A; ++c) x[fc + c] = x[n] * s[c];
                            if constexpr (DEFER) {
                                if (defer_now) {
                                    float* arow = G.avg + (size_t)j * kBoardFloats + i;
#pragma unroll
                                    for (int c = 0; c < A; ++c) {
                                        float* ap = arow + (size_t)(r0 + c) * kLdb;
                                        st_stream(ap, __fadd_rn(ld_stream(ap), __fmul_rn(x[fc + c], a.defer_w)));
                                    }
                                }
                            }
                        } else {
#pragma unroll
                            for (int c = 0; c < A; ++c) x[fc + c] = x[n];
                        }
                    } else if constexpr (SH::kind(n) == 4) {
                        constexpr int v = SH::vec_index(n);
                        if constexpr (RNR == kRnrOut) st_stream(G.rnr_reach + (size_t)j * kRnrFloats + (size_t)v * kLdb + i, x[n]);
                        else if constexpr (RNR == kRnrMix) S[v * kLdb + i] = __fmaf_rn(G.rnr_p, fm[v], x[n]);
                        else S[v * kLdb + i] = x[n];
                    } else if constexpr (RNR == kRnrMix) {
                        constexpr int f = SH::vec_index(n);
                        float m = 0.0f;
                        static_for<0, NSD>([&](auto V) {
                            constexpr int cf = SH::fold_coef(P, f, decltype(V)::value);
                            if constexpr (cf > 0) m = __fadd_rn(m, fm[decltype(V)::value]);
                            else if constexpr (cf < 0) m = __fsub_rn(m, fm[decltype(V)::value]);
                        });
                        S[(NSD + f) * kLdb + i] = __fmaf_rn(G.rnr_p, m, x[n]);
                    } else if constexpr (RNR != kRnrOut) {
                        S[(NSD + SH::vec_index(n)) * kLdb + i] = x[n];
                    }
                });
            }
        };
        {
            float gB[NOPP], gC[NOPP], xB = 0.0f, xC = 0.0f;
            p1_load_k(j, sh, 1, gB, xB);
            p1_hand(0, p1_g, p1_x0);
            p1_load_k(j, sh, 2, gC, xC);
            p1_hand(1, gB, xB);
            p1_hand(2, gC, xC);
        }
        __syncthreads();
        stamp(it, 1);
        if (kPfPhase && tid == 0) {
            if constexpr (P1ONLY) {
                if (jn < nb) prefetch_opp(jn);
            } else {
                prefetch_own(j);
            }
        }
        if constexpr (!P1ONLY) {

        mbar_wait(&bars[2], it & 1);
        float a0[NSD], a1[NSD], a2[NSD];
        double pre[NSD];
        constexpr int kQuadThreads = kLiveCards * 4;
        constexpr int kSdSplit = (NSD + 1) / 2, kFoldSplit = NF / 2;
        if (warp < (2 * kQuadThreads + 31) / 32) {
            const int grp = (tid >= kQuadThreads) ? 1 : 0;
            const int t = tid - grp * kQuadThreads;
            const bool row_live = t < kQuadThreads;
            const int lc = row_live ? (t >> 2) : (kLiveCards - 1), q = tid & 3;
            const unsigned qmask = 0xFu << (lane & 28);
            const uint2* rp = reinterpret_cast<const uint2*>(rowidx + lc * kRowPad + q * kRowSeg);
            const uint2 w0 = rp[0], w1 = rp[1], w2 = rp[2];
            const unsigned pk[6] = {w0.x, w0.y, w1.x, w1.y, w2.x, w2.y};
            int idx[kRowSeg];
#pragma unroll
            for (int e = 0; e < kRowSeg; ++e) idx[e] = (pk[e >> 1] >> ((e & 1) * 16)) & 0xffffu;
            const int v_lo = grp ? kSdSplit : 0, v_hi = grp ? NSD : kSdSplit;
#pragma unroll 1
            for (int v = v_lo; v < v_hi; ++v) {
                const float* Sv = S + v * kLdb;
                float inc[kRowSeg];
                float run = 0.0f;
#pragma unroll
                for (int e = 0; e < kRowSeg; ++e) {
                    inc[e] = run;
                    run += Sv[idx[e]];
                }
                if constexpr (kLin) {
                    double drun = (double)run;
                    drun += __shfl_xor_sync(qmask, drun, 1, 4);
                    drun += __shfl_xor_sync(qmask, drun, 2, 4);
                    if (row_live && q == 0) rowtot[v * kRowPad + lc] = drun;
                }
                float sc = run;
                float tt = __shfl_up_sync(qmask, sc, 1, 4);
                if (q >= 1) sc += tt;
                tt = __shfl_up_sync(qmask, sc, 2, 4);
                if (q >= 2) sc += tt;
                const float half = 0.5f * __shfl_sync(qmask, sc, 3, 4);
                const float off = (sc - run) - half;
                float* row = Er + v * kErVec + q * kRowSeg * kErStride + lc;
#pragma unroll
                for (int e = 0; e < kRowSeg; ++e)
                    if (row_live && q * kRowSeg + e < kErStride) row[e * kErStride] = off + inc[e];
            }
#pragma unroll 1
            for (int f = kFoldSplit * grp; f < (kLin ? 0 : kFoldSplit * grp + kFoldSplit); ++f) {
                const float* Sv = S + (NSD + f) * kLdb;
                double run = 0.0;
#pragma unroll
                for (int e = 0; e < kRowSeg; ++e) run += (double)Sv[idx[e]];
                run += __shfl_xor_sync(qmask, run, 1, 4);
                run += __shfl_xor_sync(qmask, run, 2, 4);
                if (row_live && q == 0) csd[f * kRowPad + lc] = run;
            }
        }
        __syncwarp();
        {
            const int b0 = 3 * tid;
#pragma unroll
            for (int v = 0; v < NSD; ++v) {
                const float* Sv = S + v * kLdb;
                a0[v] = (b0 < kLive) ? Sv[b0] : 0.0f;
                a1[v] = (b0 + 1 < kLive) ? Sv[b0 + 1] : 0.0f;
                a2[v] = (b0 + 2 < kLive) ? Sv[b0 + 2] : 0.0f;
                const double loc = ((double)a0[v] + (double)a1[v]) + (double)a2[v];
                double incw = loc;
#pragma unroll
                for (int o = 1; o < 32; o <<= 1) {
                    const double tt = __shfl_up_sync(0xffffffffu, incw, o);
                    if (lane >= o) incw += tt;
                }
                pre[v] = incw - loc;
                if (lane == 31) wsum[v * 16 + warp] = incw;
            }
        }
        const float mult = __ldg(G.board_mult + j);
        const double fx = (double)mult * a.fx_scale;
        const float* own_rows = tab_own + (size_t)j * kBoardFloats + (size_t)OWN0 * kLdb;
        float* reg_rows = G.regret + (size_t)j * kBoardFloats + (size_t)OWN0 * kLdb;
        float* avg_rows = G.avg + (size_t)j * kBoardFloats + (size_t)OWN0 * kLdb;
        float* pred_rows = PRED ? G.pred + (size_t)j * kBoardFloats + (size_t)OWN0 * kLdb : nullptr;
        auto p3_pos = [&](int k) -> int { return tid + k * kThreads; };
        float gA[NOWN], aA[NOWN], gB[NOWN], aB[NOWN];
        auto p3_load = [&](int k, float (&g)[NOWN], float (&av)[NOWN]) {
            const int i = min(p3_pos(k), kLive - 1);
#pragma unroll
            for (int r = 0; r < NOWN; ++r) g[r] = ld_stream(own_rows + (size_t)r * kLdb + i);
#pragma unroll
            for (int r = 0; r < NOWN; ++r) av[r] = 0.0f;
            if (read_avg) {
#pragma unroll
                for (int r = 0; r < NOWN; ++r) av[r] = ld_stream(avg_rows + (size_t)r * kLdb + i);
            }
            if constexpr (PRED) {
#pragma unroll
                for (int r = 0; r < NOWN; ++r) av[r] = ld_stream(pred_rows + (size_t)r * kLdb + i);
            }
        };
        p3_load(0, gA, aA);
        __syncthreads();
        stamp(it, 2);
        if (tid == 0 && jn < nb) {
            mbar_expect_tx(&bars[2], kRowIdxBytes);
            bulk_g2s(smem + M::kRowIdxOff, blob_g + (size_t)jn * kBlobBytes + kBlobA, kRowIdxBytes, &bars[2]);
            if constexpr (kPfPhase) prefetch_opp(jn);
        }
        auto fold_finish = [&](auto F) {
            constexpr int f = decltype(F)::value;
            double c0 = 0.0, c1 = 0.0;
            if constexpr (kLin) {
                static_for<0, NSD>([&](auto V) {
                    constexpr int v = decltype(V)::value;
                    constexpr int cf = SH::fold_coef(P, f, v);
                    if constexpr (cf != 0) {
                        const double r0 = (lane < kLiveCards) ? rowtot[v * kRowPad + lane] : 0.0;
                        const double r1 = (lane + 32 < kLiveCards) ? rowtot[v * kRowPad + lane + 32] : 0.0;
                        c0 = (cf > 0) ? c0 + r0 : c0 - r0;
                        c1 = (cf > 0) ? c1 + r1 : c1 - r1;
                    }
                });
            } else {
                c0 = (lane < kLiveCards) ? csd[f * kRowPad + lane] : 0.0;
                c1 = (lane + 32 < kLiveCards) ? csd[f * kRowPad + lane + 32] : 0.0;
            }
            double s2 = c0 + c1;
#pragma unroll
            for (int o = 16; o > 0; o >>= 1) s2 += __shfl_xor_sync(0xffffffffu, s2, o);
            if (lane == 0) tf[f] = (float)(0.5 * s2);
            if (lane < kLiveCards) cs[f * kRowPad + lane] = (float)c0;
            if (lane + 32 < kLiveCards) cs[f * kRowPad + lane + 32] = (float)c1;
        };
        {
            auto warp_totals_scan = [&](int v) {
                const double w = (lane < kWarps) ? wsum[v * 16 + lane] : 0.0;
                double sc = w;
#pragma unroll
                for (int o = 1; o < 16; o <<= 1) {
                    const double tt = __shfl_up_sync(0xffffffffu, sc, o);
                    if (lane >= o) sc += tt;
                }
                const double total = __shfl_sync(0xffffffffu, sc, kWarps - 1);
                if (lane < kWarps) wexc[v * 16 + lane] = (sc - w) - 0.5 * total;
            };
            if (warp == 0) {
#pragma unroll
                for (int v = 0; v < NSD; ++v) warp_totals_scan(v);
            } else if (warp == 1) {
                static_for<0, NF>([&](auto F) { fold_finish(F); });
            }
            __syncthreads();
            stamp(it, 3);
            const int b0 = 3 * tid;
#pragma unroll
            for (int v = 0; v < NSD; ++v) {
                float* Sv = S + v * kLdb;
                double run = pre[v] + wexc[v * 16 + warp];
                if (b0 <= kLive) Sv[b0] = (float)run;
                run += (double)a0[v];
                if (b0 + 1 <= kLive) Sv[b0 + 1] = (float)run;
                run += (double)a1[v];
                if (b0 + 2 <= kLive) Sv[b0 + 2] = (float)run;
            }
        }
        __syncthreads();
        stamp(it, 4);

        auto p3_hand = [&](int k, const float (&gown)[NOWN], float (&av)[NOWN]) {
            const int i = p3_pos(k);
            const uint64_t w = rec[i];
            const int hand = sh[i];
            long long* wacc = wp + hand;
            const int gs = (int)(w & 0x7ffu), ge = (int)((w >> 11) & 0x7ffu);
            const int lc1 = (int)((w >> 22) & 0x3fu), lc2 = (int)((w >> 28) & 0x3fu);
            const int k1 = (int)((w >> 34) & 0x3fu), t1 = (int)((w >> 40) & 0x3fu), k2 = (int)((w >> 46) & 0x3fu), t2 = (int)((w >> 52) & 0x3fu);
            const int o1 = k1 * kErStride + lc1, o1e = o1 + t1 * kErStride;
            const int o2 = k2 * kErStride + lc2, o2e = o2 + t2 * kErStride;
            float e[SH::N], br[EVAL ? SH::N : 1];
            static_for<0, SH::N>([&](auto I) {
                constexpr int n = decltype(I)::value;
                if constexpr (SH::kind(n) == 4) {
                    constexpr int v = SH::vec_index(n);
                    const float* Ev = S + v * kLdb;
                    const float* Rv = Er + v * kErVec;
                    const float all = Ev[gs] + Ev[ge];
                    const float rows = (Rv[o1] + Rv[o1e]) + (Rv[o2] + Rv[o2e]);
                    e[n] = (all - rows) * a.sc[n];
                    if constexpr (EVAL) br[n] = e[n];
                } else if constexpr (SH::kind(n) == 3) {
                    constexpr int f = SH::vec_index(n);
                    const float mass = ((tf[f] - cs[f * kRowPad + lc1]) - cs[f * kRowPad + lc2]) + S[(NSD + f) * kLdb + i];
                    e[n] = mass * a.sc[n];
                    if constexpr (EVAL) br[n] = e[n];
                }
            });
            static_for_down<0, SH::N>([&](auto I) {
                constexpr int n = decltype(I)::value;
                constexpr int A = SH::n_children(n);
                if constexpr (SH::kind(n) <= 1) {
                    constexpr int fc = SH::first_child(n);
                    if constexpr (SH::kind(n) == OPP) {
                        float v = e[fc];
#pragma unroll
                        for (int c = 1; c < A; ++c) v += e[fc + c];
                        e[n] = v;
                        if constexpr (EVAL) {
                            float b = br[fc];
#pragma unroll
                            for (int c = 1; c < A; ++c) b += br[fc + c];
                            br[n] = b;
                        }
                    } else {
                        constexpr int r0 = SH::row_of(fc) - OWN0;
                        float g[A], s[A];
#pragma unroll
                        for (int c = 0; c < A; ++c) g[c] = gown[r0 + c];
                        if constexpr (PRED) {
                            float q[A];
#pragma unroll
                            for (int c = 0; c < A; ++c) q[c] = av[r0 + c];
                            node_strategy<A>(q, 0, s);
                        } else {
                            node_strategy<A>(g, asis_own, s);
                        }
                        if (pair) {
#pragma unroll
                            for (int c = 0; c < A; ++c) av[r0 + c] = avg_step(a.m_old_due, av[r0 + c], a.m_new_due, s[c]);
                        }
                        float v = s[0] * e[fc];
#pragma unroll
                        for (int c = 1; c < A; ++c) v += s[c] * e[fc + c];
                        e[n] = v;
                        if constexpr (EVAL) {
                            float b = br[fc];
#pragma unroll
                            for (int c = 1; c < A; ++c) b = fmaxf(b, br[fc + c]);
                            br[n] = b;
                        } else {
                            if constexpr (PRED) {
#pragma unroll
                                for (int c = 0; c < A; ++c) {
                                    const float d = e[fc + c] - v;
                                    g[c] = fmaxf(d + g[c], 0.0f);
                                    st_stream(reg_rows + (size_t)(r0 + c) * kLdb + i, g[c]);
                                    st_stream(pred_rows + (size_t)(r0 + c) * kLdb + i, fmaxf(g[c] + d, 0.0f));
                                }
                            } else {
#pragma unroll
                            for (int c = 0; c < A; ++c) {
                                if constexpr (DEFER) {
                                    g[c] = __fadd_rn(__fmul_rn(a.rw, e[fc + c] - v), g[c]);
                                    if (a.disc) g[c] = __fmul_rn(g[c], (g[c] > 0.0f) ? disc[0] : disc[1]);
                                } else g[c] = fmaxf((e[fc + c] - v) + g[c], 0.0f);
                            }
                            if constexpr (!DEFER) node_strategy<A>(g, 0, s);
#pragma unroll
                            for (int c = 0; c < A; ++c) st_stream(reg_rows + (size_t)(r0 + c) * kLdb + i, g[c]);
                            if (do_avg) {
#pragma unroll
                                for (int c = 0; c < A; ++c)
                                    st_stream(avg_rows + (size_t)(r0 + c) * kLdb + i, avg_step(a.m_old, av[r0 + c], a.m_new, s[c]));
                            }
                            }
                        }
                    }
                }
            });
            atomicAdd(reinterpret_cast<unsigned long long*>(wacc), (unsigned long long)__double2ll_rn((double)e[0] * fx));
            if constexpr (EVAL)
                atomicAdd(reinterpret_cast<unsigned long long*>(wacc + kRange), (unsigned long long)__double2ll_rn((double)br[0] * fx));
        };
        p3_load(1, gB, aB);
        p3_hand(0, gA, aA);
        p3_load(2, gA, aA);
        if (p3_pos(1) < kLive) p3_hand(1, gB, aB);
        if (p3_pos(2) < kLive) p3_hand(2, gA, aA);
        }
        if (jn < nb) {
            mbar_wait(&bars[buf ^ 1], ((it + 1) >> 1) & 1);
            p1_load(jn, reinterpret_cast<const int16_t*>(smem + M::kBlobOff + (buf ^ 1) * kBlobA + kRecBytes));
        }
        __syncthreads();
        stamp(it, 5);
    }
    __syncthreads();
    unsigned long long* wt = reinterpret_cast<unsigned long long*>(G.w_total) + (EVAL ? 2 * P * kRange : 0);
    for (int h = tid; h < (EVAL ? 2 : 1) * kRange; h += kThreads) {
        const long long v = __ldcg(wp + h);
        if (v != 0) atomicAdd(wt + h, (unsigned long long)v);
    }
}

template <class SH, int P>
__global__ void __launch_bounds__(256) avg_flush_kernel(float* __restrict__ regret, float* __restrict__ avg, float m_old, float m_new) {
    constexpr size_t kBoardFloats = (size_t)SH::rows * kLdb;
    const float* reg_b = regret + (size_t)blockIdx.x * kBoardFloats;
    float* avg_b = avg + (size_t)blockIdx.x * kBoardFloats;
    for (int i = threadIdx.x; i < kLive; i += blockDim.x) {
        static_for<0, SH::N>([&](auto I) {
            constexpr int n = decltype(I)::value;
            if constexpr (SH::kind(n) == P) {
                constexpr int A = SH::n_children(n), r0 = SH::row_of(SH::first_child(n));
                float g[A], s[A];
#pragma unroll
                for (int c = 0; c < A; ++c) g[c] = ld_stream(reg_b + (size_t)(r0 + c) * kLdb + i);
                node_strategy<A>(g, 0, s);
#pragma unroll
                for (int c = 0; c < A; ++c) {
                    float* ap = avg_b + (size_t)(r0 + c) * kLdb + i;
                    st_stream(ap, avg_step(m_old, (m_old != 0.0f) ? ld_stream(ap) : 0.0f, m_new, s[c]));
                }
            }
        });
    }
}

__global__ void __launch_bounds__(256) board_tables_kernel(const int32_t* __restrict__ ranks, const uint64_t* __restrict__ board_mask,
                                                           const int8_t* __restrict__ hand_cards, int n_boards,
                                                           unsigned char* __restrict__ out) {
    __shared__ int srk[kRange];
    __shared__ short spos[kRange], sgs[kRange], sge[kRange];
    const int b = blockIdx.x;
    const uint64_t bm = board_mask[b];
    unsigned char* blob = out + (size_t)b * kBlobBytes;
    uint64_t* rec = reinterpret_cast<uint64_t*>(blob);
    int16_t* sh = reinterpret_cast<int16_t*>(blob + kRecBytes);
    int16_t* rowidx = reinterpret_cast<int16_t*>(blob + kBlobA);
    for (int h = threadIdx.x; h < kRange; h += blockDim.x) srk[h] = ranks[(size_t)b * kRange + h];
    for (int i = threadIdx.x; i < kLdb; i += blockDim.x) {
        rec[i] = 0;
        sh[i] = 0;
    }
    for (int i = threadIdx.x; i < kLiveCards * kRowPad; i += blockDim.x) rowidx[i] = (int16_t)kZeroSlot;
    __syncthreads();
    for (int h = threadIdx.x; h < kRange; h += blockDim.x) {
        const int r = srk[h];
        int lt = 0, le = 0, tb = 0;
        if (r >= 0) {
            for (int q = 0; q < kRange; ++q) {
                const int x = srk[q];
                if (x < 0) continue;
                lt += x < r;
                le += x <= r;
                tb += (x == r) && (q < h);
            }
        }
        sgs[h] = (short)(r >= 0 ? lt : -1);
        sge[h] = (short)(r >= 0 ? le : -1);
        spos[h] = (short)(r >= 0 ? lt + tb : -1);
    }
    __syncthreads();
    for (int it = threadIdx.x; it < kDeck * (kDeck - 1); it += blockDim.x) {
        const int c = it / (kDeck - 1), xr = it % (kDeck - 1);
        const int x = xr + (xr >= c);
        if (((bm >> c) | (bm >> x)) & 1ull) continue;
        const int c1 = min(c, x), c2 = max(c, x);
        const int h = c1 * (2 * kDeck - 1 - c1) / 2 + (c2 - c1 - 1);
        const int g = sgs[h], ps = spos[h];
        int lt = 0, le = 0, kpos = 0;
        for (int y = 0; y < kDeck; ++y) {
            if (y == c || ((bm >> y) & 1ull)) continue;
            const int d1 = min(c, y), d2 = max(c, y);
            const int h2 = d1 * (2 * kDeck - 1 - d1) / 2 + (d2 - d1 - 1);
            const int g2 = sgs[h2];
            lt += g2 < g;
            le += g2 <= g;
            kpos += spos[h2] < ps;
        }
        const int lc = c - __popcll(bm & ((1ull << c) - 1ull));
        rowidx[lc * kRowPad + kpos] = (int16_t)ps;
        const uint64_t fld = ((uint64_t)lc) << (c == c1 ? 22 : 28) | ((uint64_t)lt) << (c == c1 ? 34 : 46) |
                             ((uint64_t)(le - lt)) << (c == c1 ? 40 : 52);
        atomicOr(reinterpret_cast<unsigned long long*>(rec + ps), (unsigned long long)fld);
    }
    __syncthreads();
    for (int h = threadIdx.x; h < kRange; h += blockDim.x) {
        const int ps = spos[h];
        if (ps < 0) continue;
        sh[ps] = (int16_t)h;
        atomicOr(reinterpret_cast<unsigned long long*>(rec + ps),
                 (unsigned long long)((uint64_t)sgs[h] | ((uint64_t)sge[h] << 11)));
    }
}

__global__ void board_collect_kernel(const long long* __restrict__ w_total, int n_arr, const int16_t* __restrict__ sym_perm,
                                     int n_sym, double inv_scale, float* __restrict__ out, int ld) {
    const int h = blockIdx.x * blockDim.x + threadIdx.x;
    if (h >= kRange) return;
    for (int a = 0; a < n_arr; ++a) {
        long long s = 0;
        if (n_sym > 1) {
            for (int q = 0; q < n_sym; ++q) s += w_total[(size_t)a * kRange + sym_perm[(size_t)q * kRange + h]];
        } else {
            s = w_total[(size_t)a * kRange + h];
        }
        out[(size_t)a * ld + h] = (float)((double)s * inv_scale);
    }
}

__global__ void board_permute_kernel(const unsigned char* __restrict__ tables, int n_boards, int rows_per_board,
                                     const int64_t* __restrict__ row_src, const int64_t* __restrict__ row_dst, float* sorted_tab,
                                     float* natural_tab, int ld, int to_natural) {
    const int j = blockIdx.x / rows_per_board, r = blockIdx.x % rows_per_board;
    const int16_t* sh = reinterpret_cast<const int16_t*>(tables + (size_t)j * kBlobBytes + kRecBytes);
    float* srow = sorted_tab + ((size_t)row_src[2 * r] + (size_t)j * row_src[2 * r + 1]) * kLdb;
    float* nrow = natural_tab + ((size_t)row_dst[2 * r] + (size_t)j * row_dst[2 * r + 1]) * ld;
    if (to_natural) {
        for (int h = threadIdx.x; h < ld; h += blockDim.x) nrow[h] = 0.0f;
        __syncthreads();
        for (int i = threadIdx.x; i < kLive; i += blockDim.x) nrow[sh[i]] = srow[i];
    } else {
        for (int i = threadIdx.x; i < kLive; i += blockDim.x) srow[i] = nrow[sh[i]];
    }
}

__constant__ int8_t c_suit_perm[24][4] = {
    {0, 1, 2, 3}, {0, 1, 3, 2}, {0, 2, 1, 3}, {0, 2, 3, 1}, {0, 3, 1, 2}, {0, 3, 2, 1}, {1, 0, 2, 3}, {1, 0, 3, 2},
    {1, 2, 0, 3}, {1, 2, 3, 0}, {1, 3, 0, 2}, {1, 3, 2, 0}, {2, 0, 1, 3}, {2, 0, 3, 1}, {2, 1, 0, 3}, {2, 1, 3, 0},
    {2, 3, 0, 1}, {2, 3, 1, 0}, {3, 0, 1, 2}, {3, 0, 2, 1}, {3, 1, 0, 2}, {3, 1, 2, 0}, {3, 2, 0, 1}, {3, 2, 1, 0}};


__device__ __forceinline__ int hand_index(int c1, int c2) {
    return c1 * (2 * kDeck - 1 - c1) / 2 + (c2 - c1 - 1);
}

template <class SH>
__global__ void __launch_bounds__(256) policy_query_kernel(const float* __restrict__ rows, const long long* __restrict__ keys,
                                                           const int16_t* __restrict__ pos_hand, int n_cls, int iso,
                                                           const int8_t* __restrict__ boards, const int32_t* __restrict__ out_index,
                                                           unsigned long long act, int n_actions, float* __restrict__ out,
                                                           int* __restrict__ miss) {
    __shared__ short s_pos[kRange];
    __shared__ long long s_key[24];
    __shared__ int s_perm, s_cls;
    constexpr int kNDec = SH::n_dec();
    const int q = blockIdx.x, tid = threadIdx.x;
    int cards[kBoardCards];
    uint64_t bm = 0;
#pragma unroll
    for (int k = 0; k < kBoardCards; ++k) {
        cards[k] = boards[(size_t)q * kBoardCards + k];
        bm |= 1ull << cards[k];
    }
    if (tid < 24) {
        const int s = iso ? tid : 0;
        int m[kBoardCards];
#pragma unroll
        for (int k = 0; k < kBoardCards; ++k) m[k] = (cards[k] >> 2) * 4 + c_suit_perm[s][cards[k] & 3];
#pragma unroll
        for (int i = 1; i < kBoardCards; ++i)
#pragma unroll
            for (int j = i; j > 0; --j)
                if (m[j] < m[j - 1]) {
                    const int t = m[j];
                    m[j] = m[j - 1];
                    m[j - 1] = t;
                }
        long long key = 0;
#pragma unroll
        for (int k = 0; k < kBoardCards; ++k) key = key * 64 + m[k];
        s_key[tid] = key;
    }
    __syncthreads();
    if (tid == 0) {
        int best = 0;
        if (iso)
            for (int s = 1; s < 24; ++s)
                if (s_key[s] < s_key[best]) best = s;
        const long long k = s_key[best];
        int lo = 0, hi = n_cls;
        while (lo < hi) {
            const int mid = (lo + hi) >> 1;
            if (keys[mid] < k) lo = mid + 1;
            else hi = mid;
        }
        s_perm = best;
        s_cls = (lo < n_cls && keys[lo] == k) ? lo : -1;
        if (s_cls < 0) atomicExch(miss, 1);
    }
    for (int h = tid; h < kRange; h += blockDim.x) s_pos[h] = -1;
    __syncthreads();
    const int cls = s_cls, sp = s_perm;
    if (cls >= 0)
        for (int i = tid; i < kLive; i += blockDim.x) s_pos[pos_hand[(size_t)cls * kLive + i]] = (short)i;
    __syncthreads();
    const float* crow = rows + (size_t)(cls < 0 ? 0 : cls) * SH::rows * kLdb;
    for (int h = tid; h < kRange; h += blockDim.x) {
        int c1 = 0;
        while (hand_index(c1 + 1, c1 + 2) <= h) ++c1;
        const int c2 = h - hand_index(c1, c1 + 1) + c1 + 1;
        int pos = -1;
        if (cls >= 0 && !(((bm >> c1) | (bm >> c2)) & 1ull)) {
            const int m1 = (c1 >> 2) * 4 + c_suit_perm[sp][c1 & 3], m2 = (c2 >> 2) * 4 + c_suit_perm[sp][c2 & 3];
            pos = s_pos[hand_index(min(m1, m2), max(m1, m2))];
        }
#pragma unroll
        for (int d = 0; d < kNDec; ++d) {
            const int oi = out_index[(size_t)q * kNDec + d];
            if (oi < 0) continue;
            float* o = out + ((size_t)oi * kRange + h) * n_actions;
            for (int a = 0; a < n_actions; ++a) o[a] = 0.0f;
            if (pos < 0) continue;
            const int n = SH::dec_node(d), fc = SH::first_child(n);
            for (int c = fc; c < fc + SH::n_children(n); ++c)
                o[(act >> (4 * c)) & 0xF] = crow[(size_t)SH::row_of(c) * kLdb + pos];
        }
    }
}

constexpr int kTrunkThreads = 1024;

__device__ __forceinline__ float trunk_sigma(const prl_trunk_t& t, int src, int fs, int c, int A, int h) {
    if (src == PRL_STRAT_UNIFORM64) return 1.0f / (float)A;
    if (src == PRL_STRAT_AVG_SUM) {
        float tot = 0.0f;
        for (int k = 0; k < A; ++k) tot += t.avg[(size_t)(fs + k) * t.ld + h];
        return (tot == 0.0f) ? 1.0f / (float)A : t.avg[(size_t)(fs + c) * t.ld + h] / tot;
    }
    const float* tab = (src == PRL_STRAT_F32) ? t.strat : t.avg;
    return tab[(size_t)(fs + c) * t.ld + h];
}

template <bool EVAL, bool PRED = false, bool RNR = false>
__global__ void __launch_bounds__(kTrunkThreads) trunk_kernel(const prl_trunk_t t, const long long* __restrict__ w_total,
                                                              const long long* const* __restrict__ peers, int n_peers,
                                                              long long peer_offset, long long* __restrict__ w_scratch,
                                                              const int16_t* __restrict__ sym_perm, int n_sym, double inv_scale,
                                                              int p_upd, int iter, int delay, float m_old, float m_new, int algo,
                                                              float rw, const float* __restrict__ disc, float* out_expl) {
    __shared__ float ro[kRange + 2];
    __shared__ float cs[64];
    __shared__ float red[32];
    __shared__ double dred[32];
    const int tid = threadIdx.x, lane = tid & 31, warp = tid >> 5;
    const size_t N = (size_t)t.n_buf_nodes, ld = (size_t)t.ld;
    const int seat_lo = EVAL ? 0 : p_upd, seat_hi = EVAL ? 1 : p_upd;
    if (peers != nullptr) {
        for (int i = tid; i < (EVAL ? 4 : 1) * kRange; i += kTrunkThreads) {
            long long s = 0;
            for (int r = 0; r < n_peers; ++r) s += peers[r][peer_offset + i];
            w_scratch[i] = s;
        }
        __syncthreads();
        w_total = w_scratch;
    }
    for (int p = seat_lo; p <= seat_hi; ++p)
        for (int k = 0; k < (EVAL ? 2 : 1); ++k) {
            const long long* W = w_total + (size_t)(EVAL ? (2 * p + k) : 0) * kRange;
            float* dst = (k ? t.ev_br : t.ev) + ((size_t)p * N + t.chance_node) * ld;
            for (int h = tid; h < kRange; h += kTrunkThreads) {
                long long s = 0;
                if (n_sym > 1) {
                    for (int q = 0; q < n_sym; ++q) s += W[sym_perm[(size_t)q * kRange + h]];
                } else {
                    s = W[h];
                }
                dst[h] = (float)((double)s * inv_scale);
            }
        }
    for (int n = 0; n < t.n_nodes; ++n) {
        if (t.kind[n] != PRL_KIND_FOLD) continue;
        for (int p = seat_lo; p <= seat_hi; ++p) {
            const float* rg = t.reach + ((size_t)(1 - p) * N + n) * ld;
            __syncthreads();
            float part = 0.0f;
            for (int h = tid; h < kRange; h += kTrunkThreads) {
                float r = rg[h];
                if constexpr (RNR && !EVAL)
                    r = __fmaf_rn(t.rnr_p, t.reach_model[((size_t)(1 - p) * N + n) * ld + h], __fmul_rn(1.0f - t.rnr_p, r));
                ro[h] = r;
                part += r;
            }
            for (int o = 16; o > 0; o >>= 1) part += __shfl_xor_sync(0xffffffffu, part, o);
            if (lane == 0) red[warp] = part;
            __syncthreads();
            float T = 0.0f;
            for (int w = 0; w < kTrunkThreads / 32; ++w) T += red[w];
            if (tid < kDeck) {
                float acc = 0.0f;
                const int c = tid;
                for (int r = 0; r < c; ++r) acc += ro[r * (2 * kDeck - 1 - r) / 2 + c - r - 1];
                const int b0 = c * (2 * kDeck - 1 - c) / 2;
                for (int k = 0; k < kDeck - 1 - c; ++k) acc += ro[b0 + k];
                cs[c] = acc;
            }
            __syncthreads();
            const float sc = t.eq_const * t.pot[n] * 0.5f * ((t.acted_last[n] == p) ? -1.0f : 1.0f);
            float* e = t.ev + ((size_t)p * N + n) * ld;
            float* b = t.ev_br + ((size_t)p * N + n) * ld;
            for (int h = tid; h < kRange; h += kTrunkThreads) {
                const float v = (T - cs[t.hand_cards[2 * h]] - cs[t.hand_cards[2 * h + 1]] + ro[h]) * sc;
                e[h] = v;
                if (EVAL) b[h] = v;
            }
        }
    }
    __syncthreads();
    double ex[2] = {0.0, 0.0}, root_ev[2] = {0.0, 0.0}, root_br[2] = {0.0, 0.0};
    for (int h = tid; h < kRange; h += kTrunkThreads) {
        for (int n = t.n_nodes - 1; n >= 0; --n) {
            const int k = t.kind[n];
            if (k > PRL_KIND_P1) continue;
            const int A = t.n_children[n], fc = t.first_child[n], fs = t.first_slot[n];
            for (int p = seat_lo; p <= seat_hi; ++p) {
                float* ev_p = t.ev + (size_t)p * N * ld;
                float* br_p = t.ev_br + (size_t)p * N * ld;
                float v = 0.0f, b = 0.0f;
                if (k != p) {
                    for (int c = 0; c < A; ++c) v += ev_p[(size_t)(fc + c) * ld + h];
                    if (EVAL)
                        for (int c = 0; c < A; ++c) b += br_p[(size_t)(fc + c) * ld + h];
                } else {
                    for (int c = 0; c < A; ++c) v += trunk_sigma(t, t.mode[p], fs, c, A, h) * ev_p[(size_t)(fc + c) * ld + h];
                    if (EVAL) {
                        b = br_p[(size_t)fc * ld + h];
                        for (int c = 1; c < A; ++c) b = fmaxf(b, br_p[(size_t)(fc + c) * ld + h]);
                    } else if (PRED) {
                        float ssum = 0.0f;
                        for (int c = 0; c < A; ++c) {
                            float* rg = t.regret + (size_t)(fs + c) * ld + h;
                            const float d = ev_p[(size_t)(fc + c) * ld + h] - v;
                            const float r = fmaxf(d + *rg, 0.0f);
                            const float q = fmaxf(r + d, 0.0f);
                            *rg = r;
                            t.strat[(size_t)(fs + c) * ld + h] = q;
                            ssum += q;
                        }
                        const float inv = (ssum > 0.0f) ? 1.0f / ssum : 0.0f;
                        for (int c = 0; c < A; ++c) {
                            float* st = t.strat + (size_t)(fs + c) * ld + h;
                            *st = (ssum > 0.0f) ? *st * inv : 1.0f / (float)A;
                        }
                    } else {
                        float ssum = 0.0f;
                        for (int c = 0; c < A; ++c) {
                            float* rg = t.regret + (size_t)(fs + c) * ld + h;
                            const float d = ev_p[(size_t)(fc + c) * ld + h] - v;
                            float r = (algo == PRL_ALGO_CFR_PLUS) ? fmaxf(d + *rg, 0.0f) : __fadd_rn(__fmul_rn(rw, d), *rg);
                            if (disc) r = __fmul_rn(r, (r > 0.0f) ? disc[0] : disc[1]);
                            *rg = r;
                            ssum += fmaxf(r, 0.0f);
                        }
                        const float inv = (ssum > 0.0f) ? 1.0f / ssum : 0.0f;
                        for (int c = 0; c < A; ++c) {
                            const float r = fmaxf(t.regret[(size_t)(fs + c) * ld + h], 0.0f);
                            t.strat[(size_t)(fs + c) * ld + h] = (ssum > 0.0f) ? r * inv : 1.0f / (float)A;
                        }
                    }
                }
                ev_p[(size_t)n * ld + h] = v;
                if (EVAL) br_p[(size_t)n * ld + h] = b;
            }
        }
        if (EVAL) {
            for (int p = 0; p < 2; ++p)
            {
                ex[p] += (double)t.reach[((size_t)p * N) * ld + h] *
                         ((double)t.ev_br[((size_t)p * N) * ld + h] - (double)t.ev[((size_t)p * N) * ld + h]);
                if constexpr (RNR) {
                    root_ev[p] += (double)t.reach[((size_t)p * N) * ld + h] * (double)t.ev[((size_t)p * N) * ld + h];
                    root_br[p] += (double)t.reach[((size_t)p * N) * ld + h] * (double)t.ev_br[((size_t)p * N) * ld + h];
                }
            }
        } else {
            const int p = p_upd;
            float* rp = t.reach + (size_t)p * N * ld;
            for (int n = 0; n < t.n_nodes; ++n) {
                const int k = t.kind[n];
                if (k > PRL_KIND_P1) continue;
                const int A = t.n_children[n], fc = t.first_child[n], fs = t.first_slot[n];
                const float r = rp[(size_t)n * ld + h];
                for (int c = 0; c < A; ++c) {
                    float s = 1.0f;
                    if (k == p) {
                        s = t.strat[(size_t)(fs + c) * ld + h];
                        float* a = t.avg + (size_t)(fs + c) * ld + h;
                        if (PRED) *a = __fadd_rn(*a, __fmul_rn(__fmul_rn(s, r), disc[2]));
                        else if (algo != PRL_ALGO_CFR_PLUS)
                            *a = __fadd_rn(*a, __fmul_rn(__fmul_rn(s, r), disc ? disc[2] : rw));
                        else if (iter >= delay) *a = m_old * (*a) + m_new * s;
                    }
                    rp[(size_t)(fc + c) * ld + h] = s * r;
                }
            }
        }
    }
    if (EVAL) {
        for (int p = 0; p < 2; ++p) {
            double v = ex[p];
            for (int o = 16; o > 0; o >>= 1) v += __shfl_xor_sync(0xffffffffu, v, o);
            __syncthreads();
            if (lane == 0) dred[warp] = v;
            __syncthreads();
            if (tid == 0) {
                double s = 0.0;
                for (int w = 0; w < kTrunkThreads / 32; ++w) s += dred[w];
                out_expl[p] = (float)s;
            }
        }
        if constexpr (RNR) {
            for (int q = 0; q < 4; ++q) {
                double v = (q < 2) ? root_ev[q] : root_br[q - 2];
                for (int o = 16; o > 0; o >>= 1) v += __shfl_xor_sync(0xffffffffu, v, o);
                __syncthreads();
                if (lane == 0) dred[warp] = v;
                __syncthreads();
                if (tid == 0) {
                    double s = 0.0;
                    for (int w = 0; w < kTrunkThreads / 32; ++w) s += dred[w];
                    out_expl[2 + q] = (float)s;
                }
            }
        }
    }
}

template <class SH>
bool shape_matches(const prl_board_game_t* g) {
    if (g->n_local != SH::N) return false;
    for (int i = 0; i < SH::N; ++i)
        if (g->kind[i] != SH::kind(i) || g->parent[i] != SH::parent(i) || g->first_child[i] != SH::first_child(i) ||
            g->n_children[i] != SH::n_children(i))
            return false;
    return true;
}

template <class SH>
bool layout_matches(const prl_board_game_t* g) {
    for (int i = 1; i < SH::N; ++i)
        if (g->row0[i] != SH::row_of(i) || g->row_m[i] != SH::rows) return false;
    return true;
}

constexpr int kNoShape = -1000;
template <class F>
int with_shape(const prl_board_game_t* g, F&& f) {
    if (!g) return kNoShape;
    if (shape_matches<ShapeFHP>(g)) return f(ShapeFHP{});
    if (shape_matches<ShapeFHPShort>(g)) return f(ShapeFHPShort{});
    return kNoShape;
}

int default_grid() {
    static int cached[64] = {0};
    int dev = 0;
    cudaGetDevice(&dev);
    if (dev < 0 || dev >= 64) dev = 0;
    if (!cached[dev]) {
        int sms = 132;
        cudaDeviceGetAttribute(&sms, cudaDevAttrMultiProcessorCount, dev);
        cached[dev] = 2 * sms;
    }
    return cached[dev];
}

template <class SH, int P, bool EVAL, bool DEFER = false, bool P1ONLY = false, bool AVG = true, bool PRED = false, int RNR = 0>
int launch_sweep(const SweepArgs& a, int grid, cudaStream_t s) {
    auto kern = board_sweep_kernel<SH, P, EVAL, DEFER, P1ONLY, AVG, PRED, RNR>;
    constexpr int kSmemBytes = SweepSmem<SH>::kSmemBytes;
    cudaError_t e = cudaFuncSetAttribute(kern, cudaFuncAttributeMaxDynamicSharedMemorySize, kSmemBytes);
    if (e != cudaSuccess) return prl::check(e, "prl_board_sweep: shared memory opt-in");
    kern<<<grid, kThreads, kSmemBytes, s>>>(a);
    prl::count_launch();
    return 0;
}

}

extern "C" int prl_board_layout(const prl_board_game_t* shape, int32_t* out) {
    int n_local = 0;
    if (shape) {
        n_local = with_shape(shape, [](auto sh) { return decltype(sh)::N; });
        if (n_local == kNoShape) return prl::fail("prl_board_layout: the post-deal subtree has no compiled shape");
    }
    out[0] = kLive;
    out[1] = kLdb;
    out[2] = kBlobBytes;
    out[3] = kRecBytes;
    out[4] = kBlobA;
    out[5] = kLiveCards;
    out[6] = kRowPad;
    out[7] = n_local;
    return 0;
}

extern "C" int prl_board_grid(void) { return default_grid(); }

extern "C" int prl_board_rows(const prl_board_game_t* shape, int32_t* row_of, int32_t* rows_per_board) {
    const int rc = with_shape(shape, [&](auto sh) {
        using SH = decltype(sh);
        for (int i = 0; i < 16; ++i) row_of[i] = (i >= 1 && i < SH::N) ? SH::row_of(i) : -1;
        *rows_per_board = SH::rows;
        return 0;
    });
    return rc == kNoShape ? prl::fail("prl_board_rows: the post-deal subtree has no compiled shape") : rc;
}

extern "C" int prl_board_shape_ok(const prl_board_game_t* g) {
    return with_shape(g, [](auto) { return 1; }) == 1 ? 1 : 0;
}

extern "C" int prl_board_build_tables(const int32_t* ranks, const uint64_t* board_mask, const int8_t* hand_cards, int n_boards,
                                      void* blob, prl_stream_t stream) {
    if (n_boards <= 0) return 0;
    board_tables_kernel<<<n_boards, 256, 0, (cudaStream_t)stream>>>(ranks, board_mask, hand_cards, n_boards, (unsigned char*)blob);
    prl::count_launch();
    return prl::check(cudaGetLastError(), "prl_board_build_tables");
}

static int board_sweep(const prl_board_game_t* g, int p, int eval, int src_own, int src_opp, const float* trunk_reach_opp, int iter,
                       int delay, int algo, float defer_w, int p1_only, int due, int now, prl_stream_t stream) {
    if (int e = prl::check_algo(algo, g->dcfr, !eval && !p1_only, "prl_board_sweep")) return e;
    const bool pred = algo == PRL_ALGO_PCFR_PLUS;
    if (pred && !g->pred) return prl::fail("prl_board_sweep: PCFR+ needs the prediction table g->pred");
    const bool defer = !eval && algo != PRL_ALGO_CFR_PLUS;
    const bool rnr = g->rnr_reach != nullptr;
    if (rnr && algo != PRL_ALGO_CFR_PLUS) return prl::fail("prl_board_sweep: the restricted Nash response is a CFR+ form");
    if (rnr && !(g->rnr_p >= 0.0f && g->rnr_p <= 1.0f)) return prl::fail("prl_board_sweep: rnr_p must be in [0, 1]");
    if (p1_only && !defer && !rnr)
        return prl::fail("prl_board_sweep: p1_only is the average flush of Vanilla / Linear CFR or the model reach of a restricted "
                         "Nash response");
    const int layout_ok = with_shape(g, [&](auto sh) { return layout_matches<decltype(sh)>(g) ? 1 : 0; });
    if (layout_ok == kNoShape) return prl::fail("prl_board_sweep: the post-deal subtree has no compiled shape");
    if (g->n_range != kRange || g->n_deck != kDeck) return prl::fail("prl_board_sweep: 52-card deck / 1326 hands only");
    if (!layout_ok) return prl::fail("prl_board_sweep: row0 / row_m must be the board-major layout of prl_board_rows");
    if (p < 0 || p > 1) return prl::fail("prl_board_sweep: bad seat");
    if (!g->tables || !g->regret || !g->avg || !g->w_private || !g->w_total || !trunk_reach_opp)
        return prl::fail("prl_board_sweep: missing buffers");
    const bool step = now && iter >= delay;
    if (due != -1 && (due < delay || !step))
        return prl::fail("prl_board_sweep: a pending averaging step (iteration >= delay) is written with this iteration's");
    cudaStream_t s = (cudaStream_t)stream;
    const int grid = g->grid > 0 ? g->grid : default_grid();
    SweepArgs a;
    a.g = *g;
    if (pred && (eval || p1_only)) a.g.regret = g->pred;
    a.trunk_reach_opp = trunk_reach_opp;
    a.iter = iter;
    a.delay = delay;
    prl::cfrp_weights(iter, delay, &a.m_old, &a.m_new);
    a.pair = due >= 0;
    a.m_old_due = a.m_new_due = 0.0f;
    if (a.pair) prl::cfrp_weights(due, delay, &a.m_old_due, &a.m_new_due);
    a.src_own = src_own;
    a.src_opp = src_opp;
    a.rw = prl::regret_weight(algo, iter);
    a.disc = prl::dcfr_row(algo, g->dcfr, iter, !eval && !p1_only);
    a.defer_w = defer ? defer_w : 0.0f;
    a.fx_scale = (double)(1ull << g->frac_bits);
    for (int n = 0; n < 16; ++n) {
        const bool folder = n < g->n_local && g->kind[n] == PRL_KIND_FOLD && g->acted_last[n] == p;
        a.sc[n] = (n < g->n_local) ? g->eq_const * g->pot[n] * 0.5f * (folder ? -1.0f : 1.0f) : 0.0f;
    }
    if (p1_only) {
        const int rc1 = with_shape(g, [&](auto sh) {
            using SH = decltype(sh);
            if (rnr) return (p == 0) ? launch_sweep<SH, 0, false, false, true, false, false, kRnrOut>(a, grid, s)
                                     : launch_sweep<SH, 1, false, false, true, false, false, kRnrOut>(a, grid, s);
            return (p == 0) ? launch_sweep<SH, 0, false, true, true>(a, grid, s) : launch_sweep<SH, 1, false, true, true>(a, grid, s);
        });
        return rc1 ? rc1 : prl::check(cudaGetLastError(), "prl_board_sweep(flush)");
    }
    {
        char* base = reinterpret_cast<char*>(g->w_total) + (eval ? sizeof(long long) * 2 * p * kRange : 0);
        if (int e = prl::check(cudaMemsetAsync(base, 0, sizeof(long long) * (eval ? 2 : 1) * kRange, s), "prl_board_sweep: memset")) return e;
    }
    const int rc = with_shape(g, [&](auto sh) {
        using SH = decltype(sh);
        if (eval && rnr) return (p == 0) ? launch_sweep<SH, 0, true, false, false, true, false, kRnrMix>(a, grid, s)
                                         : launch_sweep<SH, 1, true, false, false, true, false, kRnrMix>(a, grid, s);
        if (eval) return (p == 0) ? launch_sweep<SH, 0, true>(a, grid, s) : launch_sweep<SH, 1, true>(a, grid, s);
        if (rnr && step) return (p == 0) ? launch_sweep<SH, 0, false, false, false, true, false, kRnrMix>(a, grid, s)
                                         : launch_sweep<SH, 1, false, false, false, true, false, kRnrMix>(a, grid, s);
        if (rnr) return (p == 0) ? launch_sweep<SH, 0, false, false, false, false, false, kRnrMix>(a, grid, s)
                                 : launch_sweep<SH, 1, false, false, false, false, false, kRnrMix>(a, grid, s);
        if (pred) return (p == 0) ? launch_sweep<SH, 0, false, true, false, true, true>(a, grid, s)
                                  : launch_sweep<SH, 1, false, true, false, true, true>(a, grid, s);
        if (defer) return (p == 0) ? launch_sweep<SH, 0, false, true>(a, grid, s) : launch_sweep<SH, 1, false, true>(a, grid, s);
        if (step) return (p == 0) ? launch_sweep<SH, 0, false>(a, grid, s) : launch_sweep<SH, 1, false>(a, grid, s);
        return (p == 0) ? launch_sweep<SH, 0, false, false, false, false>(a, grid, s)
                        : launch_sweep<SH, 1, false, false, false, false>(a, grid, s);
    });
    if (rc) return rc;
    return prl::check(cudaGetLastError(), "prl_board_sweep");
}

extern "C" int prl_board_sweep(const prl_board_game_t* g, int p, int eval, int src_own, int src_opp, const float* trunk_reach_opp,
                               int iter, int delay, int algo, float defer_w, int p1_only, prl_stream_t stream) {
    return board_sweep(g, p, eval, src_own, src_opp, trunk_reach_opp, iter, delay, algo, defer_w, p1_only, -1, 1, stream);
}

extern "C" int prl_board_update_cfrp(const prl_board_game_t* g, int p, const float* trunk_reach_opp, int iter, int delay, int due,
                                     int now, prl_stream_t stream) {
    return board_sweep(g, p, 0, 0, 0, trunk_reach_opp, iter, delay, PRL_ALGO_CFR_PLUS, 0.0f, 0, due, now, stream);
}

extern "C" int prl_board_avg_flush(const prl_board_game_t* g, int p, int due, int delay, prl_stream_t stream) {
    const int layout_ok = with_shape(g, [&](auto sh) { return layout_matches<decltype(sh)>(g) ? 1 : 0; });
    if (layout_ok != 1) return prl::fail("prl_board_avg_flush: not a compiled shape / layout");
    if (p < 0 || p > 1) return prl::fail("prl_board_avg_flush: bad seat");
    if (due < delay) return prl::fail("prl_board_avg_flush: no averaging step before iteration delay");
    if (!g->regret || !g->avg) return prl::fail("prl_board_avg_flush: missing buffers");
    if (g->n_boards <= 0) return 0;
    float m_old, m_new;
    prl::cfrp_weights(due, delay, &m_old, &m_new);
    cudaStream_t s = (cudaStream_t)stream;
    with_shape(g, [&](auto sh) {
        using SH = decltype(sh);
        if (p == 0) avg_flush_kernel<SH, 0><<<g->n_boards, 256, 0, s>>>(g->regret, g->avg, m_old, m_new);
        else avg_flush_kernel<SH, 1><<<g->n_boards, 256, 0, s>>>(g->regret, g->avg, m_old, m_new);
        return 0;
    });
    prl::count_launch();
    return prl::check(cudaGetLastError(), "prl_board_avg_flush");
}

#if PRL_BV_STAMPS
extern "C" int prl_board_stamps(int64_t* out, int32_t* shape) {
    shape[0] = kStampCtas;
    shape[1] = kStampUnits;
    shape[2] = kStampSlots;
    if (int e = prl::check(cudaMemcpyFromSymbol(out, g_stamps, sizeof(g_stamps)), "prl_board_stamps: copy")) return e;
    static const long long zeros[kStampCtas * kStampUnits * kStampSlots] = {};
    return prl::check(cudaMemcpyToSymbol(g_stamps, zeros, sizeof(g_stamps)), "prl_board_stamps: clear");
}
#endif

extern "C" int prl_board_collect(const prl_board_game_t* g, int n_arr, const int16_t* sym_perm, int n_sym, float* out, int ld,
                                 prl_stream_t stream) {
    if (!g || n_arr < 1 || n_arr > 4) return prl::fail("prl_board_collect: bad arguments");
    board_collect_kernel<<<(kRange + 255) / 256, 256, 0, (cudaStream_t)stream>>>(
        reinterpret_cast<const long long*>(g->w_total), n_arr, sym_perm, n_sym, 1.0 / (double)(1ull << g->frac_bits), out, ld);
    prl::count_launch();
    return prl::check(cudaGetLastError(), "prl_board_collect");
}

extern "C" int prl_board_permute(const prl_board_game_t* g, int rows_per_board, const int64_t* row_src, const int64_t* row_dst,
                                 float* sorted_tab, float* natural_tab, int ld, int to_natural, prl_stream_t stream) {
    if (g && with_shape(g, [](auto) { return 0; }) == kNoShape)
        return prl::fail("prl_board_permute: the post-deal subtree has no compiled shape");
    if (!g || g->n_boards <= 0 || rows_per_board <= 0) return 0;
    board_permute_kernel<<<g->n_boards * rows_per_board, 256, 0, (cudaStream_t)stream>>>(
        (const unsigned char*)g->tables, g->n_boards, rows_per_board, row_src, row_dst, sorted_tab, natural_tab, ld, to_natural);
    prl::count_launch();
    return prl::check(cudaGetLastError(), "prl_board_permute");
}

extern "C" int prl_board_policy_query(const prl_board_game_t* shape, const float* rows, const int64_t* keys, const int16_t* pos_hand,
                                      int n_cls, int iso, const int8_t* boards, int n_boards, const int32_t* out_index,
                                      uint64_t actions, int n_actions, float* out, int32_t* miss, prl_stream_t stream) {
    if (with_shape(shape, [](auto) { return 0; }) == kNoShape)
        return prl::fail("prl_board_policy_query: the post-deal subtree has no compiled shape");
    if (n_boards <= 0) return 0;
    if (!rows || !keys || !pos_hand || n_cls <= 0 || !boards || !out_index || !out || !miss)
        return prl::fail("prl_board_policy_query: missing buffers");
    if (n_actions < 1 || n_actions > 16) return prl::fail("prl_board_policy_query: 1..16 actions");
    const int rc = with_shape(shape, [&](auto sh) {
        using SH = decltype(sh);
        for (int c = 1; c < SH::N; ++c)
            if (SH::kind(SH::parent(c)) <= 1 && (int)((actions >> (4 * c)) & 0xF) >= n_actions)
                return prl::fail("prl_board_policy_query: an action id is out of range");
        policy_query_kernel<SH><<<n_boards, 256, 0, (cudaStream_t)stream>>>(rows, reinterpret_cast<const long long*>(keys), pos_hand,
                                                                            n_cls, iso, boards, out_index, (unsigned long long)actions,
                                                                            n_actions, out, reinterpret_cast<int*>(miss));
        return 0;
    });
    if (rc) return rc;
    prl::count_launch();
    return prl::check(cudaGetLastError(), "prl_board_policy_query");
}

extern "C" int prl_board_trunk(const prl_board_game_t* g, const prl_trunk_t* t, int eval, int p, int n_sym, const int16_t* sym_perm,
                               int iter, int delay, float* out_expl, const int64_t* const* peers, int n_peers,
                               int64_t peer_offset, int64_t* w_scratch, int algo, prl_stream_t stream) {
    if (int e = prl::check_algo(algo, g ? g->dcfr : nullptr, !eval, "prl_board_trunk")) return e;
    if (!g || !t || t->n_nodes < 1 || t->n_nodes > 8) return prl::fail("prl_board_trunk: 1..8 trunk nodes");
    const float rw = prl::regret_weight(algo, iter);
    const bool pred = algo == PRL_ALGO_PCFR_PLUS && !eval;
    const float* disc = pred ? g->dcfr + 3 * (size_t)iter : prl::dcfr_row(algo, g->dcfr, iter, !eval);
    if (with_shape(g, [](auto) { return 0; }) == kNoShape) return prl::fail("prl_board_trunk: the post-deal subtree has no compiled shape");
    if (t->n_range != kRange || g->n_deck != kDeck) return prl::fail("prl_board_trunk: 52-card deck / 1326 hands only");
    if (eval && !out_expl) return prl::fail("prl_board_trunk: out_expl missing");
    for (int n = 0; n < t->n_nodes; ++n)
        if (t->kind[n] == PRL_KIND_SHOWDOWN || t->kind[n] == PRL_KIND_SHOWDOWN_ALLIN)
            return prl::fail("prl_board_trunk: showdowns before the deal are not supported");
    float m_old, m_new;
    prl::cfrp_weights(iter, delay, &m_old, &m_new);
    const double inv_scale = 1.0 / (double)(1ull << g->frac_bits);
    const long long* w = reinterpret_cast<const long long*>(g->w_total);
    if (peers && (n_peers < 1 || !w_scratch)) return prl::fail("prl_board_trunk: peer sum needs n_peers >= 1 and w_scratch");
    const long long* const* pp = reinterpret_cast<const long long* const*>(peers);
    long long* ws = reinterpret_cast<long long*>(w_scratch);
    const bool rnr = t->reach_model != nullptr;
    if (rnr && (algo != PRL_ALGO_CFR_PLUS || !(t->rnr_p >= 0.0f && t->rnr_p <= 1.0f)))
        return prl::fail("prl_board_trunk: the restricted Nash response is a CFR+ form with rnr_p in [0, 1]");
    if (rnr)
        (eval ? trunk_kernel<true, false, true> : trunk_kernel<false, false, true>)<<<1, kTrunkThreads, 0, (cudaStream_t)stream>>>(
            *t, w, pp, n_peers, (long long)peer_offset, ws, sym_perm, n_sym, inv_scale, eval ? -1 : p, iter, delay, m_old, m_new, algo,
            rw, disc, out_expl);
    else if (eval)
        trunk_kernel<true><<<1, kTrunkThreads, 0, (cudaStream_t)stream>>>(*t, w, pp, n_peers, (long long)peer_offset, ws, sym_perm, n_sym,
                                                                       inv_scale, -1, iter, delay, m_old, m_new, algo, rw, disc, out_expl);
    else if (pred)
        trunk_kernel<false, true><<<1, kTrunkThreads, 0, (cudaStream_t)stream>>>(*t, w, pp, n_peers, (long long)peer_offset, ws, sym_perm,
                                                                              n_sym, inv_scale, p, iter, delay, m_old, m_new, algo, rw, disc,
                                                                              out_expl);
    else
        trunk_kernel<false><<<1, kTrunkThreads, 0, (cudaStream_t)stream>>>(*t, w, pp, n_peers, (long long)peer_offset, ws, sym_perm, n_sym,
                                                                        inv_scale, p, iter, delay, m_old, m_new, algo, rw, disc, out_expl);
    prl::count_launch();
    return prl::check(cudaGetLastError(), "prl_board_trunk");
}
```

Measured before the change: 64.83.

## Stream compact per-board index and rebuild row index and hand ids in kernel

The sweep kernel now bulk-loads a smaller per-board index (records, packed rank positions, board mask) in place of the full blob plus a separate row-index copy. Hand ids are recomputed from live-card tables derived from the board mask, and the shared-memory row index is rebuilt during phase 1. This cuts global-to-shared traffic and drops one mbarrier and bulk copy per board. In exchange it adds integer work per hand (popcount loops, index arithmetic) and scattered shared-memory stores, and it changes the ABI.

```diff
diff --git a/include/pokerrl_b200.h b/include/pokerrl_b200.h
--- a/include/pokerrl_b200.h
+++ b/include/pokerrl_b200.h
@@ -9,7 +9,7 @@
 
 typedef void* prl_stream_t;
 
-#define PRL_ABI_VERSION 10
+#define PRL_ABI_VERSION 11
 
 enum {
     PRL_KIND_P0 = 0,
@@ -157,6 +157,7 @@
     float* pred;
     float* rnr_reach;
     float rnr_p;
+    const void* index;
 } prl_board_game_t;
 
 int prl_board_layout(const prl_board_game_t* shape, int32_t* out);
@@ -165,7 +166,8 @@
 int prl_board_rows(const prl_board_game_t* shape, int32_t* row_of, int32_t* rows_per_board);
 
 int prl_board_build_tables(const int32_t* ranks, const uint64_t* board_mask, const int8_t* hand_cards, int n_boards,
-                           void* blob, prl_stream_t stream);
+                           void* blob, void* index, prl_stream_t stream);
+int prl_board_rebuild_tables(const void* index, int n_boards, void* blob, prl_stream_t stream);
 
 int prl_board_sweep(const prl_board_game_t* g, int p, int eval, int src_own, int src_opp, const float* trunk_reach_opp,
                     int iter, int delay, int algo, float defer_w, int p1_only, prl_stream_t stream);
diff --git a/pokerrl_b200/_native.py b/pokerrl_b200/_native.py
--- a/pokerrl_b200/_native.py
+++ b/pokerrl_b200/_native.py
@@ -6,7 +6,7 @@
 
 KIND_P0, KIND_P1, KIND_CHANCE, KIND_FOLD, KIND_SHOWDOWN, KIND_SHOWDOWN_ALLIN = range(6)
 ALGO_VANILLA, ALGO_CFR_PLUS, ALGO_LINEAR, ALGO_DCFR, ALGO_PCFR_PLUS = 0, 1, 2, 3, 4
-ABI_VERSION = 10
+ABI_VERSION = 11
 STRAT_F32, STRAT_UNIFORM64, STRAT_AVG_F64, STRAT_AVG_SUM, STRAT_AVG_F32 = range(5)
 
 
@@ -44,7 +44,7 @@
                 ("row0", C.c_int64 * 16), ("row_m", C.c_int32 * 16),
                 ("tables", C.c_void_p), ("board_prob", C.c_void_p), ("board_mult", C.c_void_p), ("regret", C.c_void_p),
                 ("avg", C.c_void_p), ("w_private", C.c_void_p), ("w_total", C.c_void_p), ("dcfr", C.c_void_p), ("pred", C.c_void_p),
-                ("rnr_reach", C.c_void_p), ("rnr_p", C.c_float)]
+                ("rnr_reach", C.c_void_p), ("rnr_p", C.c_float), ("index", C.c_void_p)]
 
 
 class PrlTrunk(C.Structure):
@@ -134,7 +134,8 @@
     L.prl_board_rows.argtypes = [gp, C.POINTER(C.c_int32), C.POINTER(C.c_int32)]
     L.prl_board_rows.restype = C.c_int
     L.prl_board_shape_ok.argtypes = [gp]
-    L.prl_board_build_tables.argtypes = [C.c_void_p, C.c_void_p, C.c_void_p, C.c_int, C.c_void_p, C.c_void_p]
+    L.prl_board_build_tables.argtypes = [C.c_void_p, C.c_void_p, C.c_void_p, C.c_int, C.c_void_p, C.c_void_p, C.c_void_p]
+    L.prl_board_rebuild_tables.argtypes = [C.c_void_p, C.c_int, C.c_void_p, C.c_void_p]
     L.prl_board_sweep.argtypes = [gp, C.c_int, C.c_int, C.c_int, C.c_int, C.c_void_p, C.c_int, C.c_int, C.c_int, C.c_float, C.c_int,
                                   C.c_void_p]
     L.prl_board_update_cfrp.argtypes = [gp, C.c_int, C.c_void_p, C.c_int, C.c_int, C.c_int, C.c_int, C.c_void_p]
@@ -147,7 +148,8 @@
     L.prl_board_trunk.restype = C.c_int
     L.prl_board_policy_query.argtypes = [gp, C.c_void_p, C.c_void_p, C.c_void_p, C.c_int, C.c_int, C.c_void_p, C.c_int,
                                          C.c_void_p, C.c_uint64, C.c_int, C.c_void_p, C.c_void_p, C.c_void_p]
-    for f in ("prl_board_layout", "prl_board_grid", "prl_board_shape_ok", "prl_board_build_tables", "prl_board_sweep",
+    for f in ("prl_board_layout", "prl_board_grid", "prl_board_shape_ok", "prl_board_build_tables", "prl_board_rebuild_tables",
+              "prl_board_sweep",
               "prl_board_update_cfrp", "prl_board_avg_flush", "prl_board_collect", "prl_board_permute", "prl_board_policy_query"):
         getattr(L, f).restype = C.c_int
     ep = C.POINTER(PrlEnvCfg)
diff --git a/pokerrl_b200/board_engine.py b/pokerrl_b200/board_engine.py
--- a/pokerrl_b200/board_engine.py
+++ b/pokerrl_b200/board_engine.py
@@ -16,10 +16,10 @@
 
 
 def board_layout(g=None):
-    out = (C.c_int32 * 8)()
+    out = (C.c_int32 * 10)()
     nat.call("prl_board_layout", C.byref(g) if g is not None else None, out)
     return dict(n_live=out[0], ldb=out[1], blob=out[2], sh_off=out[3], rows_off=out[4], live_cards=out[5],
-                row_pad=out[6], n_local=out[7])
+                row_pad=out[6], n_local=out[7], index=out[8], mask_off=out[9])
 
 
 def _stream(dev):
@@ -67,7 +67,7 @@
     return mask
 
 
-def build_board_blobs(rules, boards, t_blob, dev):
+def build_board_blobs(rules, boards, t_blob, t_index, dev):
     from pokerrl_b200.hand_eval import hand_rank_all_hands_on_given_boards
     boards = np.ascontiguousarray(boards, np.int8)
     nb = boards.shape[0]
@@ -79,7 +79,8 @@
         n = min(CH, nb - i)
         ranks = hand_rank_all_hands_on_given_boards(boards[i:i + n], device=dev)
         nat.call("prl_board_build_tables", C.c_void_p(ranks.data_ptr()), C.c_void_p(t_mask[i:i + n].data_ptr()),
-                 C.c_void_p(t_hc.data_ptr()), n, C.c_void_p(t_blob[i:i + n].data_ptr()), _stream(dev))
+                 C.c_void_p(t_hc.data_ptr()), n, C.c_void_p(t_blob[i:i + n].data_ptr()),
+                 C.c_void_p(t_index[i:i + n].data_ptr()), _stream(dev))
 
 
 def _decision_locals(st):
@@ -181,14 +182,16 @@
     def _setup_boards(self, capacity):
         dev, n = self.device, max(capacity, 1)
         self.t_blob = torch.empty((n, self.L["blob"]), dtype=torch.uint8, device=dev)
+        self.t_index = torch.empty((n, self.L["index"]), dtype=torch.uint8, device=dev)
         self.t_prob = torch.zeros(n, dtype=torch.float32, device=dev)
         self.t_mult = torch.zeros(n, dtype=torch.float32, device=dev)
         g = self.g
         g.tables, g.board_prob, g.board_mult = self.t_blob.data_ptr(), self.t_prob.data_ptr(), self.t_mult.data_ptr()
+        g.index = self.t_index.data_ptr()
 
     def _load_boards(self, boards, prob, mult):
         n = boards.shape[0]
-        build_board_blobs(self.rules, boards, self.t_blob, self.device)
+        build_board_blobs(self.rules, boards, self.t_blob, self.t_index, self.device)
         self.t_prob[:n].copy_(torch.from_numpy(np.ascontiguousarray(prob, np.float32)))
         self.t_mult[:n].copy_(torch.from_numpy(np.ascontiguousarray(mult, np.float32)))
         self.g.n_boards = n
@@ -580,8 +583,9 @@
         sh = self._share
         if sh.n_boards != capacity or not np.array_equal(sh.boards, self.boards) or sh.device != self.device:
             raise ValueError("share_boards: another board spec or device")
-        self.t_blob, self.t_prob, self.t_mult = sh.t_blob, sh.t_prob, sh.t_mult
+        self.t_blob, self.t_index, self.t_prob, self.t_mult = sh.t_blob, sh.t_index, sh.t_prob, sh.t_mult
         self.g.tables, self.g.board_prob, self.g.board_mult = sh.g.tables, sh.g.board_prob, sh.g.board_mult
+        self.g.index = sh.g.index
 
     def _load_boards(self, boards, prob, mult):
         if self._share is None:
@@ -692,7 +696,7 @@
             self._setup(game_cls, self.env_args, self.spec, 0)
             L, rpb, g = self.L, self.rows_per_board, self.g
             n_dec = len(_decision_locals(self.st))
-            self.bytes_per_board = (L["blob"] + rpb * L["ldb"] * 4 + rpb * self.ld * 4 + n_dec * self.R * n_actions * 4
+            self.bytes_per_board = (L["blob"] + L["index"] + rpb * L["ldb"] * 4 + rpb * self.ld * 4 + n_dec * self.R * n_actions * 4
                                     + self.R * 4)
             if chunk is None:
                 free, _ = torch.cuda.mem_get_info(dev)
diff --git a/pokerrl_b200/csrc/cfr_board.cu b/pokerrl_b200/csrc/cfr_board.cu
--- a/pokerrl_b200/csrc/cfr_board.cu
+++ b/pokerrl_b200/csrc/cfr_board.cu
@@ -24,7 +24,11 @@
 constexpr int kRowIdxBytes = kLiveCards * kRowPad * 2;
 constexpr int kBlobA = kRecBytes + kShBytes;
 constexpr int kBlobBytes = kBlobA + kRowIdxBytes;
-static_assert(kBlobA % 16 == 0 && kRowIdxBytes % 16 == 0, "bulk copies move multiples of 16 bytes");
+constexpr int kRankOff = kRecBytes;
+constexpr int kMaskOff = kRankOff + kShBytes - 8;
+constexpr int kIndexBytes = kRecBytes + kShBytes;
+static_assert(kBlobA % 16 == 0 && kIndexBytes % 16 == 0, "bulk copies move multiples of 16 bytes");
+static_assert(kMaskOff % 8 == 0 && kMaskOff >= kRankOff + 2 * kLive, "the mask lies past the last hand's ranks");
 
 #ifndef PRL_BV_STAMPS
 #define PRL_BV_STAMPS 0
@@ -142,15 +146,16 @@
     static constexpr int kErOff = kSOff + kNVec * kLdb * 4;
     static constexpr int kErBytes = ((SH::n_sd * kErVec * 4) + 15) & ~15;
     static constexpr int kBlobOff = kErOff + kErBytes;
-    static constexpr int kRowIdxOff = kBlobOff + 2 * kBlobA;
+    static constexpr int kRowIdxOff = kBlobOff + 2 * kIndexBytes;
     static constexpr int kCsOff = kRowIdxOff + kRowIdxBytes;
     static constexpr int kCsdOff = kCsOff + SH::n_fold * kRowPad * 4;
     static constexpr int kMiscOff = kCsdOff + SH::n_fold * kRowPad * 8;
     static constexpr int kMiscBytes = (SH::n_sd * 16 + SH::n_sd * 16) * 8 + 8 * 4;
     static constexpr int kRowTotOff = kMiscOff + kMiscBytes;
     static constexpr int kRowTotBytes = SH::n_sd * kRowPad * 8;
-    static constexpr int kBarOff = kRowTotOff + kRowTotBytes;
-    static constexpr int kSmemBytes = kBarOff + 32;
+    static constexpr int kCardOff = kRowTotOff + kRowTotBytes;
+    static constexpr int kBarOff = kCardOff + 2 * kRowPad;
+    static constexpr int kSmemBytes = kBarOff + 24;
     static_assert(kBlobOff % 16 == 0 && kRowIdxOff % 16 == 0 && kCsdOff % 8 == 0 && kMiscOff % 8 == 0 && kRowTotOff % 8 == 0 &&
                       kBarOff % 8 == 0, "alignment");
     static_assert(2 * (kSmemBytes + 1024) <= 233472, "two CTAs per SM (228 KB of shared memory per H100 SM)");
@@ -248,6 +253,30 @@
 
 __device__ __forceinline__ float ld_stream(const float* p) { return __ldcs(p); }
 __device__ __forceinline__ void st_stream(float* p, float v) { __stcs(p, v); }
+
+__device__ __forceinline__ int hand_index(int c1, int c2) {
+    return c1 * (2 * kDeck - 1 - c1) / 2 + (c2 - c1 - 1);
+}
+
+__device__ __forceinline__ int live_card(uint64_t bm, int lc) {
+    int c = lc;
+    for (;;) {
+        const int n = lc + __popcll(bm & ((2ull << c) - 1ull));
+        if (n == c) return c;
+        c = n;
+    }
+}
+
+__device__ __forceinline__ int index_hand(uint64_t w, const uint8_t* card) {
+    return hand_index(card[(w >> 22) & 0x3f], card[(w >> 28) & 0x3f]);
+}
+__device__ __forceinline__ int index_hand(uint64_t w, uint64_t bm) {
+    return hand_index(live_card(bm, (int)((w >> 22) & 0x3f)), live_card(bm, (int)((w >> 28) & 0x3f)));
+}
+__device__ __forceinline__ void index_rows(uint64_t w, unsigned rk, int i, int16_t* rowidx) {
+    rowidx[((w >> 22) & 0x3f) * kRowPad + (rk & 0x3f)] = (int16_t)i;
+    rowidx[((w >> 28) & 0x3f) * kRowPad + ((rk >> 6) & 0x3f)] = (int16_t)i;
+}
 
 constexpr int kRnrMix = 1, kRnrOut = 2;
 template <class SH, int P, bool EVAL, bool DEFER = false, bool P1ONLY = false, bool AVG = true, bool PRED = false, int RNR = 0>
@@ -266,7 +295,8 @@
     double* wexc = wsum + NSD * 16;
     float* tf = reinterpret_cast<float*>(wexc + NSD * 16);
     uint64_t* bars = reinterpret_cast<uint64_t*>(smem + M::kBarOff);
-    const int16_t* rowidx = reinterpret_cast<const int16_t*>(smem + M::kRowIdxOff);
+    int16_t* rowidx = reinterpret_cast<int16_t*>(smem + M::kRowIdxOff);
+    uint8_t* cards = smem + M::kCardOff;
     double* rowtot = reinterpret_cast<double*>(smem + M::kRowTotOff);
     constexpr bool kLin = !EVAL;
 
@@ -279,7 +309,7 @@
     constexpr int OPP0 = (P == 0) ? SH::rows_of_seat(0) : 0;
     constexpr int NOWN = SH::rows_of_seat(P), NOPP = SH::rows_of_seat(OPP);
     constexpr size_t kBoardFloats = (size_t)ROWS * kLdb;
-    const unsigned char* blob_g = reinterpret_cast<const unsigned char*>(G.tables);
+    const unsigned char* index_g = reinterpret_cast<const unsigned char*>(G.index);
     const float* tab_opp = PRED ? G.pred : (RNR == kRnrOut || (EVAL && a.src_opp >= 1)) ? G.avg : G.regret;
     const float* tab_own = (EVAL && a.src_own >= 1) ? G.avg : G.regret;
     const int asis_opp = (RNR == kRnrOut || (EVAL && a.src_opp == 1)) ? 1 : 0, asis_own = (EVAL && a.src_own == 1) ? 1 : 0;
@@ -287,17 +317,17 @@
     const bool do_avg = !EVAL && !DEFER && AVG && a.iter >= a.delay;
     const bool pair = do_avg && a.pair;
     const bool defer_now = DEFER && a.defer_w != 0.0f;
-    float* disc = reinterpret_cast<float*>(smem + M::kBarOff + 3 * sizeof(uint64_t));
+    float* disc = reinterpret_cast<float*>(smem + M::kBarOff + 2 * sizeof(uint64_t));
     const bool read_avg = do_avg && (pair ? a.m_old_due : a.m_old) != 0.0f;
 
     long long* wp = reinterpret_cast<long long*>(G.w_private) + (size_t)blockIdx.x * 2 * kRange;
     for (int h = tid; h < 2 * kRange; h += kThreads) wp[h] = 0;
     for (int v = 0; v < M::kNVec; ++v)
         for (int i = kLive + tid; i < kLdb; i += kThreads) S[v * kLdb + i] = 0.0f;
+    if (tid < kLiveCards) rowidx[tid * kRowPad + kRowLen] = rowidx[tid * kRowPad + kRowLen + 1] = (int16_t)kZeroSlot;
     if (tid == 0) {
         mbar_init(&bars[0], 1);
         mbar_init(&bars[1], 1);
-        mbar_init(&bars[2], 1);
         fence_async_shared();
         if (DEFER && a.disc) {
             disc[0] = a.disc[0];
@@ -325,47 +355,56 @@
         if constexpr (PRED) bulk_prefetch_l2(G.pred + (size_t)jj * kBoardFloats + (size_t)OWN0 * kLdb, NOWN * kLdb * 4);
     };
     if (tid == 0 && j < nb) {
-        mbar_expect_tx(&bars[0], kBlobA);
-        bulk_g2s(smem + M::kBlobOff, blob_g + (size_t)j * kBlobBytes, kBlobA, &bars[0]);
-        if (!P1ONLY) {
-            mbar_expect_tx(&bars[2], kRowIdxBytes);
-            bulk_g2s(smem + M::kRowIdxOff, blob_g + (size_t)j * kBlobBytes + kBlobA, kRowIdxBytes, &bars[2]);
-        }
+        mbar_expect_tx(&bars[0], kIndexBytes);
+        bulk_g2s(smem + M::kBlobOff, index_g + (size_t)j * kIndexBytes, kIndexBytes, &bars[0]);
         if constexpr (kPfPhase) prefetch_opp(j);
         else prefetch_rows(j);
     }
+    auto card_table = [&](int b) {
+        if (tid < kLiveCards)
+            cards[b * kRowPad + tid] =
+                (uint8_t)live_card(*reinterpret_cast<const uint64_t*>(smem + M::kBlobOff + b * kIndexBytes + kMaskOff), tid);
+    };
+    if (j < nb) {
+        mbar_wait(&bars[0], 0);
+        card_table(0);
+    }
+    __syncthreads();
 
     float p1_g[NOPP], p1_x0;
-    auto p1_load_k = [&](int jj, const int16_t* sh_jj, int k, float (&g)[NOPP], float& x0) {
+    auto p1_load_k = [&](int jj, int hand, int k, float (&g)[NOPP], float& x0) {
         const int i = min(tid + k * kThreads, kLive - 1);
         const float* rows = tab_opp + (size_t)jj * kBoardFloats + (size_t)OPP0 * kLdb + i;
 #pragma unroll
         for (int r = 0; r < NOPP; ++r) g[r] = ld_stream(rows + (size_t)r * kLdb);
-        x0 = __ldg(a.trunk_reach_opp + sh_jj[i]);
+        x0 = __ldg(a.trunk_reach_opp + hand);
     };
-    auto p1_load = [&](int jj, const int16_t* sh_jj) { p1_load_k(jj, sh_jj, 0, p1_g, p1_x0); };
+    auto p1_load = [&](int jj, const unsigned char* ix) {
+        p1_load_k(jj, index_hand(reinterpret_cast<const uint64_t*>(ix)[tid], *reinterpret_cast<const uint64_t*>(ix + kMaskOff)), 0,
+                  p1_g, p1_x0);
+    };
 
     for (int it = 0; j < nb; j += gridDim.x, ++it) {
         const int buf = it & 1;
-        const unsigned char* blob = smem + M::kBlobOff + buf * kBlobA;
-        const uint64_t* rec = reinterpret_cast<const uint64_t*>(blob);
-        const int16_t* sh = reinterpret_cast<const int16_t*>(blob + kRecBytes);
+        const unsigned char* ix = smem + M::kBlobOff + buf * kIndexBytes;
+        const uint64_t* rec = reinterpret_cast<const uint64_t*>(ix);
+        const uint16_t* rank = reinterpret_cast<const uint16_t*>(ix + kRankOff);
+        const uint8_t* card = cards + buf * kRowPad;
+        auto own_hand = [&](int k) { return (tid + k * kThreads < kLive) ? index_hand(rec[tid + k * kThreads], card) : 0; };
         const int jn = j + gridDim.x;
         stamp(it, 0);
         if (tid == 0 && jn < nb) {
-            mbar_expect_tx(&bars[buf ^ 1], kBlobA);
-            bulk_g2s(smem + M::kBlobOff + (buf ^ 1) * kBlobA, blob_g + (size_t)jn * kBlobBytes, kBlobA, &bars[buf ^ 1]);
+            mbar_expect_tx(&bars[buf ^ 1], kIndexBytes);
+            bulk_g2s(smem + M::kBlobOff + (buf ^ 1) * kIndexBytes, index_g + (size_t)jn * kIndexBytes, kIndexBytes, &bars[buf ^ 1]);
             if constexpr (!kPfPhase) prefetch_rows(jn);
         }
         const float prob = __ldg(G.board_prob + j);
-        if (it == 0) {
-            mbar_wait(&bars[buf], 0);
-            p1_load(j, sh);
-        }
+        if (it == 0) p1_load(j, ix);
 
         auto p1_hand = [&](int k, const float (&gk)[NOPP], float x0k) {
             const int i = tid + k * kThreads;
             if (i < kLive) {
+                if constexpr (!P1ONLY) index_rows(rec[i], rank[i], i, rowidx);
                 float x[SH::N];
                 x[0] = x0k * prob;
                 float fm[RNR == kRnrMix ? NSD : 1];
@@ -422,9 +461,9 @@
         };
         {
             float gB[NOPP], gC[NOPP], xB = 0.0f, xC = 0.0f;
-            p1_load_k(j, sh, 1, gB, xB);
+            p1_load_k(j, own_hand(1), 1, gB, xB);
             p1_hand(0, p1_g, p1_x0);
-            p1_load_k(j, sh, 2, gC, xC);
+            p1_load_k(j, own_hand(2), 2, gC, xC);
             p1_hand(1, gB, xB);
             p1_hand(2, gC, xC);
         }
@@ -439,7 +478,6 @@
         }
         if constexpr (!P1ONLY) {
 
-        mbar_wait(&bars[2], it & 1);
         float a0[NSD], a1[NSD], a2[NSD];
         double pre[NSD];
         constexpr int kQuadThreads = kLiveCards * 4;
@@ -542,10 +580,8 @@
         p3_load(0, gA, aA);
         __syncthreads();
         stamp(it, 2);
-        if (tid == 0 && jn < nb) {
-            mbar_expect_tx(&bars[2], kRowIdxBytes);
-            bulk_g2s(smem + M::kRowIdxOff, blob_g + (size_t)jn * kBlobBytes + kBlobA, kRowIdxBytes, &bars[2]);
-            if constexpr (kPfPhase) prefetch_opp(jn);
+        if constexpr (kPfPhase) {
+            if (tid == 0 && jn < nb) prefetch_opp(jn);
         }
         auto fold_finish = [&](auto F) {
             constexpr int f = decltype(F)::value;
@@ -610,7 +646,7 @@
         auto p3_hand = [&](int k, const float (&gown)[NOWN], float (&av)[NOWN]) {
             const int i = p3_pos(k);
             const uint64_t w = rec[i];
-            const int hand = sh[i];
+            const int hand = index_hand(w, card);
             long long* wacc = wp + hand;
             const int gs = (int)(w & 0x7ffu), ge = (int)((w >> 11) & 0x7ffu);
             const int lc1 = (int)((w >> 22) & 0x3fu), lc2 = (int)((w >> 28) & 0x3fu);
@@ -719,7 +755,8 @@
         }
         if (jn < nb) {
             mbar_wait(&bars[buf ^ 1], ((it + 1) >> 1) & 1);
-            p1_load(jn, reinterpret_cast<const int16_t*>(smem + M::kBlobOff + (buf ^ 1) * kBlobA + kRecBytes));
+            p1_load(jn, smem + M::kBlobOff + (buf ^ 1) * kIndexBytes);
+            card_table(buf ^ 1);
         }
         __syncthreads();
         stamp(it, 5);
@@ -758,8 +795,9 @@
 
 __global__ void __launch_bounds__(256) board_tables_kernel(const int32_t* __restrict__ ranks, const uint64_t* __restrict__ board_mask,
                                                            const int8_t* __restrict__ hand_cards, int n_boards,
-                                                           unsigned char* __restrict__ out) {
+                                                           unsigned char* __restrict__ out, unsigned char* __restrict__ index_out) {
     __shared__ int srk[kRange];
+    __shared__ unsigned srow[kRange];
     __shared__ short spos[kRange], sgs[kRange], sge[kRange];
     const int b = blockIdx.x;
     const uint64_t bm = board_mask[b];
@@ -767,7 +805,10 @@
     uint64_t* rec = reinterpret_cast<uint64_t*>(blob);
     int16_t* sh = reinterpret_cast<int16_t*>(blob + kRecBytes);
     int16_t* rowidx = reinterpret_cast<int16_t*>(blob + kBlobA);
-    for (int h = threadIdx.x; h < kRange; h += blockDim.x) srk[h] = ranks[(size_t)b * kRange + h];
+    for (int h = threadIdx.x; h < kRange; h += blockDim.x) {
+        srk[h] = ranks[(size_t)b * kRange + h];
+        srow[h] = 0;
+    }
     for (int i = threadIdx.x; i < kLdb; i += blockDim.x) {
         rec[i] = 0;
         sh[i] = 0;
@@ -813,6 +854,7 @@
         const uint64_t fld = ((uint64_t)lc) << (c == c1 ? 22 : 28) | ((uint64_t)lt) << (c == c1 ? 34 : 46) |
                              ((uint64_t)(le - lt)) << (c == c1 ? 40 : 52);
         atomicOr(reinterpret_cast<unsigned long long*>(rec + ps), (unsigned long long)fld);
+        atomicOr(&srow[h], (unsigned)kpos << (c == c1 ? 0 : 6));
     }
     __syncthreads();
     for (int h = threadIdx.x; h < kRange; h += blockDim.x) {
@@ -821,6 +863,34 @@
         sh[ps] = (int16_t)h;
         atomicOr(reinterpret_cast<unsigned long long*>(rec + ps),
                  (unsigned long long)((uint64_t)sgs[h] | ((uint64_t)sge[h] << 11)));
+    }
+    __syncthreads();
+    unsigned char* ix = index_out + (size_t)b * kIndexBytes;
+    uint16_t* rk = reinterpret_cast<uint16_t*>(ix + kRankOff);
+    for (int i = threadIdx.x; i < kLdb; i += blockDim.x) reinterpret_cast<uint64_t*>(ix)[i] = rec[i];
+    for (int i = kLive + threadIdx.x; i < kMaskOff / 2 - kRankOff / 2; i += blockDim.x) rk[i] = 0;
+    for (int h = threadIdx.x; h < kRange; h += blockDim.x)
+        if (spos[h] >= 0) rk[spos[h]] = (uint16_t)srow[h];
+    if (threadIdx.x == 0) *reinterpret_cast<uint64_t*>(ix + kMaskOff) = bm;
+}
+
+__global__ void __launch_bounds__(256) board_index_tables_kernel(const unsigned char* __restrict__ index, unsigned char* __restrict__ out) {
+    __shared__ uint8_t card[kRowPad];
+    const unsigned char* ix = index + (size_t)blockIdx.x * kIndexBytes;
+    unsigned char* blob = out + (size_t)blockIdx.x * kBlobBytes;
+    const uint64_t* rec = reinterpret_cast<const uint64_t*>(ix);
+    const uint16_t* rank = reinterpret_cast<const uint16_t*>(ix + kRankOff);
+    int16_t* rowidx = reinterpret_cast<int16_t*>(blob + kBlobA);
+    if (threadIdx.x < kLiveCards) {
+        card[threadIdx.x] = (uint8_t)live_card(*reinterpret_cast<const uint64_t*>(ix + kMaskOff), threadIdx.x);
+        rowidx[threadIdx.x * kRowPad + kRowLen] = rowidx[threadIdx.x * kRowPad + kRowLen + 1] = (int16_t)kZeroSlot;
+    }
+    __syncthreads();
+    for (int i = threadIdx.x; i < kLdb; i += blockDim.x) {
+        const uint64_t w = rec[i];
+        reinterpret_cast<uint64_t*>(blob)[i] = w;
+        reinterpret_cast<int16_t*>(blob + kRecBytes)[i] = (int16_t)(i < kLive ? index_hand(w, card) : 0);
+        if (i < kLive) index_rows(w, rank[i], i, rowidx);
     }
 }
 
@@ -859,11 +929,6 @@
     {0, 1, 2, 3}, {0, 1, 3, 2}, {0, 2, 1, 3}, {0, 2, 3, 1}, {0, 3, 1, 2}, {0, 3, 2, 1}, {1, 0, 2, 3}, {1, 0, 3, 2},
     {1, 2, 0, 3}, {1, 2, 3, 0}, {1, 3, 0, 2}, {1, 3, 2, 0}, {2, 0, 1, 3}, {2, 0, 3, 1}, {2, 1, 0, 3}, {2, 1, 3, 0},
     {2, 3, 0, 1}, {2, 3, 1, 0}, {3, 0, 1, 2}, {3, 0, 2, 1}, {3, 1, 0, 2}, {3, 1, 2, 0}, {3, 2, 0, 1}, {3, 2, 1, 0}};
-
-
-__device__ __forceinline__ int hand_index(int c1, int c2) {
-    return c1 * (2 * kDeck - 1 - c1) / 2 + (c2 - c1 - 1);
-}
 
 template <class SH>
 __global__ void __launch_bounds__(256) policy_query_kernel(const float* __restrict__ rows, const long long* __restrict__ keys,
@@ -1222,6 +1287,8 @@
     out[5] = kLiveCards;
     out[6] = kRowPad;
     out[7] = n_local;
+    out[8] = kIndexBytes;
+    out[9] = kMaskOff;
     return 0;
 }
 
@@ -1242,11 +1309,21 @@
 }
 
 extern "C" int prl_board_build_tables(const int32_t* ranks, const uint64_t* board_mask, const int8_t* hand_cards, int n_boards,
-                                      void* blob, prl_stream_t stream) {
+                                      void* blob, void* index, prl_stream_t stream) {
     if (n_boards <= 0) return 0;
-    board_tables_kernel<<<n_boards, 256, 0, (cudaStream_t)stream>>>(ranks, board_mask, hand_cards, n_boards, (unsigned char*)blob);
+    if (!blob || !index) return prl::fail("prl_board_build_tables: missing buffers");
+    board_tables_kernel<<<n_boards, 256, 0, (cudaStream_t)stream>>>(ranks, board_mask, hand_cards, n_boards, (unsigned char*)blob,
+                                                                   (unsigned char*)index);
     prl::count_launch();
     return prl::check(cudaGetLastError(), "prl_board_build_tables");
+}
+
+extern "C" int prl_board_rebuild_tables(const void* index, int n_boards, void* blob, prl_stream_t stream) {
+    if (n_boards <= 0) return 0;
+    if (!index || !blob) return prl::fail("prl_board_rebuild_tables: missing buffers");
+    board_index_tables_kernel<<<n_boards, 256, 0, (cudaStream_t)stream>>>((const unsigned char*)index, (unsigned char*)blob);
+    prl::count_launch();
+    return prl::check(cudaGetLastError(), "prl_board_rebuild_tables");
 }
 
 static int board_sweep(const prl_board_game_t* g, int p, int eval, int src_own, int src_opp, const float* trunk_reach_opp, int iter,
@@ -1266,7 +1343,7 @@
     if (g->n_range != kRange || g->n_deck != kDeck) return prl::fail("prl_board_sweep: 52-card deck / 1326 hands only");
     if (!layout_ok) return prl::fail("prl_board_sweep: row0 / row_m must be the board-major layout of prl_board_rows");
     if (p < 0 || p > 1) return prl::fail("prl_board_sweep: bad seat");
-    if (!g->tables || !g->regret || !g->avg || !g->w_private || !g->w_total || !trunk_reach_opp)
+    if (!g->index || !g->regret || !g->avg || !g->w_private || !g->w_total || !trunk_reach_opp)
         return prl::fail("prl_board_sweep: missing buffers");
     const bool step = now && iter >= delay;
     if (due != -1 && (due < delay || !step))
```

After: 65.15, median of 6. About the same (+0.5%).
